# skeskinen/bert.cpp

Hardware: AMD Instinct MI355X
Metric: sentences/sec (seq_len=128) (higher is better)
Workload: dtype f16; 1 GPU; all-MiniLM-L6-v2 f16, batch=256 seq_len=128; per_gpu_batch=256, global_batch=256, seq_len=128, weights=f16, parallelism=dp1 (replicated weights, sharded sentences)

## Files before the change

bert.cpp_amd/csrc/device.h:

```cpp
#pragma once
#include "kernels.h"

#include <cstdio>
#include <type_traits>
#include <utility>

namespace bert_hip {

typedef _Float16 f16x2 __attribute__((ext_vector_type(2)));
typedef _Float16 f16x4 __attribute__((ext_vector_type(4)));
typedef _Float16 f16x8 __attribute__((ext_vector_type(8)));
typedef float f32x2 __attribute__((ext_vector_type(2)));
typedef float f32x4 __attribute__((ext_vector_type(4)));
typedef float f32x8 __attribute__((ext_vector_type(8)));
typedef float f32x16 __attribute__((ext_vector_type(16)));
typedef uint32_t u32x4 __attribute__((ext_vector_type(4)));
typedef uint32_t u32x16 __attribute__((ext_vector_type(16)));
typedef int32_t i32x4 __attribute__((ext_vector_type(4)));
typedef int32_t i32x16 __attribute__((ext_vector_type(16)));

template <int... I, class F>
__device__ __forceinline__ void static_for_impl(std::integer_sequence<int, I...>, F &&f) {
    (f(std::integral_constant<int, I>{}), ...);
}
template <int N, class F>
__device__ __forceinline__ void static_for(F &&f) { static_for_impl(std::make_integer_sequence<int, N>{}, f); }

#define AS_GLOBAL(p) ((const __attribute__((address_space(1))) void *)(p))
#define AS_LDS(p) ((__attribute__((address_space(3))) void *)(p))
template <class T>
using lds_cptr = const __attribute__((address_space(3))) T *;


#ifdef BERT_HIP_TIMELINE
static __device__ unsigned long long g_timeline[1024 * 256];
#define TL_STAMP(i) do { const int tl_i = (i); if (threadIdx.x == 0 && tl_i < 256) g_timeline[(blockIdx.x & 1023) * 256 + tl_i] = __builtin_readcyclecounter(); } while (0)
#define TL_STAMP_AT(sel, i) do { const int tl_i = (i); if ((sel) && tl_i < 256) g_timeline[(blockIdx.x & 1023) * 256 + tl_i] = __builtin_readcyclecounter(); } while (0)
#define TL_REALTIME_AT(sel, i) do { const int tl_i = (i); if ((sel) && tl_i < 256) g_timeline[(blockIdx.x & 1023) * 256 + tl_i] = __builtin_amdgcn_s_memrealtime(); } while (0)
#define TL_DUMP(cond, nstamps) do {                                                                          \
    static int tl_shots = 0;                                                                                  \
    if ((cond) && tl_shots++ == 20) {                                                                         \
        (void)hipDeviceSynchronize();                                                                         \
        static unsigned long long tl_h[1024 * 256];                                                           \
        (void)hipMemcpyFromSymbol(tl_h, HIP_SYMBOL(g_timeline), sizeof(tl_h));                                \
        const int tl_n = (nstamps) < 256 ? (nstamps) : 256;                                                   \
        for (int b : {0, 1, 100, 255}) {                                                                      \
            fprintf(stderr, "timeline wg %3d:", b);                                                           \
            for (int i = 1; i < tl_n; ++i) fprintf(stderr, " %llu", tl_h[b * 256 + i] - tl_h[b * 256 + i - 1]); \
            fprintf(stderr, "  total %llu\n", tl_h[b * 256 + tl_n - 1] - tl_h[b * 256]);                      \
        }                                                                                                     \
    }                                                                                                         \
} while (0)
#define TL_DUMP_RAW(cond, nstamps) do {                                                                      \
    static int tl_shots = 0;                                                                                  \
    if ((cond) && tl_shots++ == 20) {                                                                         \
        (void)hipDeviceSynchronize();                                                                         \
        static unsigned long long tl_h[1024 * 256];                                                           \
        (void)hipMemcpyFromSymbol(tl_h, HIP_SYMBOL(g_timeline), sizeof(tl_h));                                \
        for (int b : {0, 100}) {                                                                              \
            fprintf(stderr, "rawtimeline wg %3d:", b);                                                        \
            for (int i = 0; i < (nstamps); ++i)                                                               \
                fprintf(stderr, " %lld", tl_h[b * 256 + i] ? (long long)(tl_h[b * 256 + i] - tl_h[b * 256]) : -1LL); \
            fprintf(stderr, "\n");                                                                            \
        }                                                                                                     \
    }                                                                                                         \
} while (0)
#else
#define TL_DUMP_RAW(cond, nstamps) do { } while (0)
#define TL_REALTIME_AT(sel, i) do { } while (0)
#define TL_STAMP(i) do { } while (0)
#define TL_STAMP_AT(sel, i) do { } while (0)
#define TL_DUMP(cond, nstamps) do { } while (0)
#endif

__device__ __forceinline__ unsigned lds_addr(const void *p) {
    return (unsigned)(size_t)(__attribute__((address_space(3))) const char *)p;
}
template <bool MEMORY, int OFF, class V = f16x8>
__device__ __forceinline__ V lds_read_b128(unsigned addr) {
    static_assert(sizeof(V) == 16, "ds_read_b128 reads 16 bytes");
    static_assert(OFF >= 0 && OFF < 65536, "ds offset field is 16 bits");
    V v;
    if constexpr (MEMORY) asm volatile("ds_read_b128 %0, %1 offset:%2" : "=v"(v) : "v"(addr), "n"(OFF) : "memory");
    else asm volatile("ds_read_b128 %0, %1 offset:%2" : "=v"(v) : "v"(addr), "n"(OFF));
    return v;
}
template <class V>
__device__ __forceinline__ void landed(V &v) { asm volatile("" : "+v"(v)); }
template <int VM>
__device__ __forceinline__ void dma_barrier() {
    asm volatile("s_waitcnt vmcnt(%0) lgkmcnt(0)\n\ts_barrier" : : "n"(VM) : "memory");
}

__device__ __forceinline__ int off64(int row, int chunk) { return row * 128 + ((chunk ^ ((row >> 1) & 7)) << 4); }

__device__ __forceinline__ float rounded_f32(float v) {
    asm("" : "+v"(v));
    return v;
}

__device__ __forceinline__ void xor32_pair(float &a, float &b) {
    asm("s_nop 1\n\tv_permlane32_swap_b32 %0, %1\n\ts_nop 1" : "+v"(a), "+v"(b));
}
__device__ __forceinline__ f16x8 result_to_operand_fragment(const f16x8 &v) {
    const u32x4 d = __builtin_bit_cast(u32x4, v);
    uint32_t d0 = d[0], d1 = d[1], d2 = d[2], d3 = d[3];
    asm("s_nop 1\n\tv_permlane32_swap_b32 %0, %2\n\tv_permlane32_swap_b32 %1, %3\n\ts_nop 1" : "+v"(d0), "+v"(d1), "+v"(d2), "+v"(d3));
    return __builtin_bit_cast(f16x8, u32x4{d0, d1, d2, d3});
}
constexpr int ctx_edge_offset(int nq) { return nq * 4096 > 80 * 1024 ? nq * 4096 : 80 * 1024; }
__device__ __forceinline__ float xor32_sum(float v) { float a = v, b = v; xor32_pair(a, b); return a + b; }
__device__ __forceinline__ float xor32_max(float v) { float a = v, b = v; xor32_pair(a, b); return __builtin_fmaxf(a, b); }
__device__ __forceinline__ float wave_sum_f32(float v) {
    v = xor32_sum(v);
    v += __builtin_bit_cast(float, __builtin_amdgcn_ds_swizzle(__builtin_bit_cast(int, v), (16 << 10) | 0x1F));
    v += __builtin_bit_cast(float, __builtin_amdgcn_ds_swizzle(__builtin_bit_cast(int, v), (8 << 10) | 0x1F));
    v += __builtin_bit_cast(float, __builtin_amdgcn_ds_swizzle(__builtin_bit_cast(int, v), (4 << 10) | 0x1F));
    v += __builtin_bit_cast(float, __builtin_amdgcn_mov_dpp(__builtin_bit_cast(int, v), 0x4E, 0xF, 0xF, true));
    v += __builtin_bit_cast(float, __builtin_amdgcn_mov_dpp(__builtin_bit_cast(int, v), 0xB1, 0xF, 0xF, true));
    return v;
}

#ifndef BERT_HIP_EXP16
#define BERT_HIP_EXP16 0
#endif
#if BERT_HIP_EXP16
typedef u32x4 sm_arg_t;
typedef u32x4 sm_exp_t;
__device__ __forceinline__ sm_arg_t softmax_args4(float s0, float s1, float s2, float s3, float s4, float s5, float s6, float s7, float sc, float m) {
    uint32_t a0, a1, a2, a3;
    asm("v_fma_mixlo_f16 %0, %4, %12, -%13\n\t"
        "v_fma_mixlo_f16 %1, %6, %12, -%13\n\t"
        "v_fma_mixlo_f16 %2, %8, %12, -%13\n\t"
        "v_fma_mixlo_f16 %3, %10, %12, -%13\n\t"
        "v_fma_mixhi_f16 %0, %5, %12, -%13\n\t"
        "v_fma_mixhi_f16 %1, %7, %12, -%13\n\t"
        "v_fma_mixhi_f16 %2, %9, %12, -%13\n\t"
        "v_fma_mixhi_f16 %3, %11, %12, -%13"
        : "=&v"(a0), "=&v"(a1), "=&v"(a2), "=&v"(a3)
        : "v"(s0), "v"(s1), "v"(s2), "v"(s3), "v"(s4), "v"(s5), "v"(s6), "v"(s7), "s"(sc), "v"(m));
    return u32x4{a0, a1, a2, a3};
}
__device__ __forceinline__ sm_exp_t softmax_exp4(sm_arg_t a) {
    uint32_t p0, p1, p2, p3;
    asm("v_exp_f16_e32 %0, %4\n\t"
        "v_exp_f16_e32 %1, %5\n\t"
        "v_exp_f16_e32 %2, %6\n\t"
        "v_exp_f16_e32 %3, %7\n\t"
        "v_exp_f16_sdwa %0, %4 dst_sel:WORD_1 dst_unused:UNUSED_PRESERVE src0_sel:WORD_1\n\t"
        "v_exp_f16_sdwa %1, %5 dst_sel:WORD_1 dst_unused:UNUSED_PRESERVE src0_sel:WORD_1\n\t"
        "v_exp_f16_sdwa %2, %6 dst_sel:WORD_1 dst_unused:UNUSED_PRESERVE src0_sel:WORD_1\n\t"
        "v_exp_f16_sdwa %3, %7 dst_sel:WORD_1 dst_unused:UNUSED_PRESERVE src0_sel:WORD_1\n\t"
        "s_nop 0"
        : "=&v"(p0), "=&v"(p1), "=&v"(p2), "=&v"(p3)
        : "v"(a[0]), "v"(a[1]), "v"(a[2]), "v"(a[3]));
    return u32x4{p0, p1, p2, p3};
}
__device__ __forceinline__ void softmax_sum4(sm_exp_t p, float &psum) {
    const f16x2 one = {(_Float16)1.0f, (_Float16)1.0f};
#pragma unroll
    for (int e = 0; e < 4; ++e) {
        const uint32_t pe = p[e];
        psum = __builtin_amdgcn_fdot2(__builtin_bit_cast(f16x2, pe), one, psum, false);
    }
}
__device__ __forceinline__ f16x8 softmax_pack(sm_exp_t p) { return __builtin_bit_cast(f16x8, p); }
#else
typedef f32x8 sm_arg_t;
typedef f32x8 sm_exp_t;
__device__ __forceinline__ sm_arg_t softmax_args4(float s0, float s1, float s2, float s3, float s4, float s5, float s6, float s7, float sc, float m) {
    const float s[8] = {s0, s1, s2, s3, s4, s5, s6, s7};
    f32x8 a;
#pragma unroll
    for (int e = 0; e < 8; ++e) a[e] = __builtin_fmaf(s[e], sc, -m);
    return a;
}
__device__ __forceinline__ sm_exp_t softmax_exp4(sm_arg_t a) {
    f32x8 p;
#pragma unroll
    for (int e = 0; e < 8; ++e) p[e] = __builtin_amdgcn_exp2f(a[e]);
    return p;
}
__device__ __forceinline__ void softmax_sum4(sm_exp_t p, float &psum) {
#pragma unroll
    for (int e = 0; e < 8; ++e) psum += p[e];
}
__device__ __forceinline__ f16x8 softmax_pack(sm_exp_t p) {
    f16x8 pf;
#pragma unroll
    for (int e = 0; e < 8; ++e) pf[e] = (_Float16)p[e];
    return pf;
}
#endif
__device__ __forceinline__ f16x8 softmax_p8(float s0, float s1, float s2, float s3, float s4, float s5, float s6, float s7, float sc,
                                            float m, float &psum) {
    const sm_exp_t p = softmax_exp4(softmax_args4(s0, s1, s2, s3, s4, s5, s6, s7, sc, m));
    softmax_sum4(p, psum);
    return softmax_pack(p);
}
__device__ __forceinline__ f16x2 gelu_pk16h(f16x2 xh) {
    const float c1 = -2.0f * 0.79788456080286535588f * 1.44269504088896340736f;
    const f16x2 C1 = {(_Float16)c1, (_Float16)c1}, C2 = {(_Float16)(c1 * 0.044715f), (_Float16)(c1 * 0.044715f)};
    const f16x2 one = {(_Float16)1.0f, (_Float16)1.0f};
    const f16x2 t = (xh * xh * C2 + C1) * xh;
    const f16x2 e = {(_Float16)__builtin_exp2f16(t[0]), (_Float16)__builtin_exp2f16(t[1])};
    const f16x2 d = e + one;
    const f16x2 r = {(_Float16)__builtin_amdgcn_rcph(d[0]), (_Float16)__builtin_amdgcn_rcph(d[1])};
    return xh * r;
}
__device__ __forceinline__ f16x2 gelu_pk16(float a0, float a1) { return gelu_pk16h(f16x2{(_Float16)a0, (_Float16)a1}); }

__device__ __forceinline__ void layernorm_scale(float s1, float s2, float inv_h, float &rstd, float &nmr) {
    const float mean = s1 * inv_h, ex2 = s2 * inv_h;
    const float t = fmaxf(__builtin_fmaf(-mean, mean, ex2), 0.f) + 1e-5f;
    const float r = __builtin_amdgcn_rsqf(t);
    rstd = r * __builtin_fmaf(-0.5f * t, r * r, 1.5f);
    nmr = -mean * rstd;
}

struct RawBlock { uint4 q; unsigned sc; };
template <int WT>
__device__ __forceinline__ RawBlock q4_load_block(const uint4 *qs, const void *sc, size_t index) {
    RawBlock r;
    r.q = qs[index];
    r.sc = WT == GW_Q4_0 ? (unsigned)((const unsigned short *)sc)[index] : ((const unsigned *)sc)[index];
    return r;
}
template <int WT>
struct Q4Expansion {
    f16x2 d2, m2, off;
    unsigned magic, sel01, sel23;
    __device__ __forceinline__ explicit Q4Expansion(unsigned sc) {
        if (WT == GW_Q4_0) {
            const _Float16 d = __builtin_bit_cast(_Float16, (unsigned short)(sc & 0xffffu));
            d2 = (f16x2){d, d};
            m2 = (f16x2){(_Float16)0, (_Float16)0};
        } else {
            const f16x2 dm = __builtin_bit_cast(f16x2, sc);
            d2 = (f16x2){dm[0], dm[0]};
            m2 = (f16x2){dm[1], dm[1]};
        }
        unsigned offb;
        asm volatile("v_mov_b32 %0, 0x64646464" : "=v"(magic));
        asm volatile("s_mov_b32 %0, 0x04010400" : "=s"(sel01));
        asm volatile("s_mov_b32 %0, 0x04030402" : "=s"(sel23));
        if (WT == GW_Q4_0) asm volatile("s_mov_b32 %0, 0x64086408" : "=s"(offb));
        else asm volatile("s_mov_b32 %0, 0x64006400" : "=s"(offb));
        off = __builtin_bit_cast(f16x2, offb);
    }
    template <bool Q_FIRST>
    __device__ __forceinline__ void four(unsigned word, bool high, unsigned &o0, unsigned &o1) const {
        const unsigned n4 = (high ? (word >> 4) : word) & 0x0f0f0f0fu;
        f16x2 v0 = __builtin_bit_cast(f16x2, __builtin_amdgcn_perm(magic, n4, sel01)) - off;
        f16x2 v1 = __builtin_bit_cast(f16x2, __builtin_amdgcn_perm(magic, n4, sel23)) - off;
        if (WT == GW_Q4_0) { v0 = v0 * d2; v1 = v1 * d2; }
        else if (Q_FIRST) { v0 = __builtin_elementwise_fma(v0, d2, m2); v1 = __builtin_elementwise_fma(v1, d2, m2); }
        else { v0 = __builtin_elementwise_fma(d2, v0, m2); v1 = __builtin_elementwise_fma(d2, v1, m2); }
        o0 = __builtin_bit_cast(unsigned, v0);
        o1 = __builtin_bit_cast(unsigned, v1);
    }
};
template <int WT, bool PERM, class ChunkPtr>
__device__ __forceinline__ void q4_expand_block(const RawBlock &r, ChunkPtr chunk_ptr) {
    const unsigned w[4] = {r.q.x, r.q.y, r.q.z, r.q.w};
    const Q4Expansion<WT> x(r.sc);
#pragma unroll
    for (int h = 0; h < 2; ++h)
#pragma unroll
        for (int pr = 0; pr < 2; ++pr) {
            uint4 out;
            x.template four<false>(w[PERM ? pr : 2 * pr], h, out.x, out.y);
            x.template four<false>(w[PERM ? pr + 2 : 2 * pr + 1], h, out.z, out.w);
            *(uint4 *)chunk_ptr(2 * h + pr) = out;
        }
}
template <int WT>
__device__ __forceinline__ uint4 q4_expand_chunk(const RawBlock &r, int c) {
    const Q4Expansion<WT> x(r.sc);
    const bool high = c >= 2;
    const unsigned w0 = (c & 1) ? r.q.z : r.q.x, w1 = (c & 1) ? r.q.w : r.q.y;
    uint4 out;
    x.template four<true>(w0, high, out.x, out.y);
    x.template four<true>(w1, high, out.z, out.w);
    return out;
}

template <bool PAIR, int NT, class Run, class Landed>
__device__ __forceinline__ void layernorm_runs_of(Run x, Landed landed, const float *gamma, const float *beta, int hi, f16x4 (&y)[4 * NT][4]) {
    constexpr int H = 128 * NT;
    constexpr int AHEAD = 2;
    f32x4 gv[AHEAD + 1][4], bv[AHEAD + 1][4];
    auto request = [&](int n) __attribute__((always_inline)) {
#pragma unroll
        for (int g = 0; g < 4; ++g) {
            gv[n % (AHEAD + 1)][g] = *(const f32x4 *)(gamma + 32 * n + 8 * g + 4 * hi);
            bv[n % (AHEAD + 1)][g] = *(const f32x4 *)(beta + 32 * n + 8 * g + 4 * hi);
        }
    };
#pragma unroll
    for (int n = 0; n < AHEAD; ++n) request(n);
    landed();
    float s1 = 0.f, s2 = 0.f;
    auto add_block = [&](float &a1, float &a2, int n) __attribute__((always_inline)) {
#pragma unroll
        for (int g = 0; g < 4; ++g) {
            const f32x4 v = x(n, g);
#pragma unroll
            for (int e = 0; e < 4; ++e) { a1 += v[e]; a2 = __builtin_fmaf(v[e], v[e], a2); }
        }
    };
    if constexpr (PAIR) {
        float t1[2] = {0.f, 0.f}, t2[2] = {0.f, 0.f};
#pragma unroll
        for (int role = 0; role < 2; ++role)
#pragma unroll
            for (int b = 0; b < 2 * NT; ++b) add_block(t1[role], t2[role], (b >> 1) * 4 + role * 2 + (b & 1));
#pragma unroll
        for (int role = 0; role < 2; ++role) { t1[role] += __shfl_xor(t1[role], 32); t2[role] += __shfl_xor(t2[role], 32); }
        s1 = t1[0] + t1[1]; s2 = t2[0] + t2[1];
    } else {
#pragma unroll
        for (int n = 0; n < 4 * NT; ++n) add_block(s1, s2, n);
        s1 += __shfl_xor(s1, 32); s2 += __shfl_xor(s2, 32);
    }
    float rstd, nmr;
    layernorm_scale(s1, s2, 1.0f / H, rstd, nmr);
    asm volatile("" ::: "memory");
#pragma unroll
    for (int n = 0; n < 4 * NT; ++n) {
        if (n + AHEAD < 4 * NT) request(n + AHEAD);
        __builtin_amdgcn_sched_barrier(0);
#pragma unroll
        for (int g = 0; g < 4; ++g) {
            const f32x4 v = x(n, g), gq = gv[n % (AHEAD + 1)][g], bq = bv[n % (AHEAD + 1)][g];
            f32x4 r;
#pragma unroll
            for (int e = 0; e < 4; ++e) r[e] = __builtin_fmaf(v[e], gq[e] * rstd, __builtin_fmaf(gq[e], nmr, bq[e]));
            asm("" : "+v"(r));
#pragma unroll
            for (int e = 0; e < 4; ++e) y[n][g][e] = (_Float16)r[e];
        }
        __builtin_amdgcn_sched_barrier(0);
    }
}

template <bool PAIR, int NT>
__device__ __forceinline__ void layernorm_runs(const float *row, const float *gamma, const float *beta, int hi, f16x4 (&y)[4 * NT][4]) {
    f32x4 x[4 * NT][4];
#pragma unroll
    for (int n = 0; n < 4 * NT; ++n)
#pragma unroll
        for (int g = 0; g < 4; ++g) x[n][g] = *(const f32x4 *)(row + 32 * n + 8 * g + 4 * hi);
    layernorm_runs_of<PAIR, NT>([&](int n, int g) __attribute__((always_inline)) { return x[n][g]; }, [] {}, gamma, beta, hi, y);
}

}
```

bert.cpp_amd/csrc/engine.h:

```cpp
#pragma once
#include <hip/hip_runtime.h>

#include <cstdint>
#include <functional>
#include <memory>
#include <string>
#include <vector>

#include "kernels.h"
#include "model_file.h"
#include "options.h"
#include "profiler.h"
#include "weights.h"

namespace bert_hip {

class Engine {
public:
    static Engine *create(const ModelFile &mf, int device, std::string &err);
    ~Engine();

    int eval_packed_host(const int32_t *tokens, const int32_t *cu_seqlens, int n_sentences, float *embeddings,
                         std::string &err, float *d_embeddings = nullptr);
    int eval_packed_device(const int32_t *d_tokens, const int32_t *d_cu, int n_sentences, int n_tokens, int max_len,
                           float *d_out, hipStream_t stream, float *d_hidden, std::string &err,
                           const int2 *d_windows = nullptr, int n_windows = 0, int window_slots = 0,
                           int pool_mode = -1);
    static void build_windows(const int32_t *cu_seqlens, int n_sentences, std::vector<int2> &windows, int slots);
    int eval_hidden(const int32_t *tokens, int n_tokens, float *hidden, float *embedding, std::string &err);

    bool reserve(int n_tokens, int n_sentences, std::string &err);
    int check(std::string &err);
    void set_option(const std::string &key, const std::string &value);
    void profile_enable(bool on) { prof_.enable(on); }
    std::string profile_report();
    void timed_launch(const char *name, double flops, hipStream_t s, const std::function<void()> &f);

    const HParams &hparams() const { return hp_; }
    const EngineOptions &options() const { return opt_; }
    int device() const { return device_; }
    hipStream_t stream() const { return stream_; }

private:
    Engine() = default;
    bool ensure_workspace(int t_pad, int n_sentences, std::string &err);

    enum class Route { F32, LATENCY, ONE_LAUNCH, FOLDED, LAYERED };
    enum class Family { GEMM256, MFMA, NAIVE, F32 };
    struct LayerPlan {
        bool qkv2 = false;
        bool tail = false;
        bool planes = false;
        Family qkv = Family::NAIVE, o = Family::NAIVE, ffi = Family::NAIVE, ffo = Family::NAIVE;
    };
    struct Plan {
        const int32_t *tokens, *cu;
        int B, T, max_len, t_pad, slots, pool_mode;
        float *out, *hidden;
        hipStream_t s;
        const int2 *windows;
        int n_windows;
        Route route = Route::LAYERED;
        bool build_windows = false;
        const int *n_windows_dev = nullptr;
        std::vector<LayerPlan> layers;
    };
    Plan plan(const int32_t *d_tokens, const int32_t *d_cu, int B, int T, int max_len, float *d_out, hipStream_t s, float *d_hidden,
              const int2 *d_windows, int n_windows, int slots, int pool_mode) const;
    bool forward_f32(const Plan &p, std::string &err);
    void forward_latency(const Plan &p);
    void forward_one_launch(const Plan &p);
    bool forward_folded(const Plan &p, std::string &err);
    bool forward_layers(const Plan &p, std::string &err);
    bool gemm(const Plan &p, const char *name, Family f, const GemmWeightStore &W, const void *A, const float *bias, const void *resid, void *C,
              int epi, std::string &err, const GemmLnFold *ln = nullptr);
    void attention(const Plan &p);
    void tap(const Plan &p, int idx);
    template <class F> void timed(const char *name, double flops, hipStream_t s, F &&f) { prof_.timed(name, flops, s, f); }

    HParams hp_;
    int device_ = 0;
    EngineOptions opt_;
    std::unique_ptr<ModelWeights> w_;
    LaunchProfiler prof_;

    DevBuf x_, qkv_, ctx_, y_, ff_, v32_, d_tokens_, d_cu_, d_out_, d_hidden_, status_, windows_;
    DevBuf ln_stats1_, ln_stats2_, ln_rows1_, ln_rows2_;
    hipStream_t stream_ = nullptr;
    hipEvent_t busy_ = nullptr;
    struct HostSlot {
        char *h_in = nullptr, *d_in_host = nullptr;
        float *h_out = nullptr, *d_out_host = nullptr;
        size_t h_in_cap = 0, h_out_cap = 0;
        DevBuf d_in, d_out;
        hipEvent_t done = nullptr;
    } slot_[2];
};

}
```

bert.cpp_amd/csrc/engine.hip:

```cpp
#include "engine.h"

#include <algorithm>
#include <cstdio>
#include <cstdlib>
#include <chrono>
#include <cstring>
#include <system_error>
#include <thread>

namespace bert_hip {

Engine *Engine::create(const ModelFile &mf, int device, std::string &err) {
    int ndev = 0;
    if (hipGetDeviceCount(&ndev) != hipSuccess || ndev <= 0) {
        err = "no HIP device available (this library needs an AMD GPU; there is no CPU fallback)";
        return nullptr;
    }
    if (device < 0 || device >= ndev) { err = "HIP device ordinal " + std::to_string(device) + " out of range"; return nullptr; }
    std::unique_ptr<Engine> e(new Engine);
    e->hp_ = mf.hp;
    e->device_ = device;
    if (hipSetDevice(e->device_) != hipSuccess) { err = "hipSetDevice failed"; return nullptr; }
    hipDeviceProp_t prop;
    if (hipGetDeviceProperties(&prop, e->device_) != hipSuccess) { err = "hipGetDeviceProperties failed"; return nullptr; }
    if (strncmp(prop.gcnArchName, "gfx950", 6) != 0) {
        err = std::string("unsupported GPU architecture '") + prop.gcnArchName + "' (kernels are built for gfx950 / MI355X only)";
        return nullptr;
    }
    e->opt_ = EngineOptions::from_env(mf.hp);
    LoadOptions lo;
    lo.naive = e->opt_.gemm_naive; lo.expand_q4 = e->opt_.q4_expand; lo.ln_fold = e->opt_.ln_fold;
    e->w_ = ModelWeights::load(mf, lo, err);
    if (!e->w_ || !e->status_.alloc(16, err)) return nullptr;
    if (hipStreamCreateWithFlags(&e->stream_, hipStreamNonBlocking) != hipSuccess) { err = "hipStreamCreate failed"; return nullptr; }
    if (hipEventCreateWithFlags(&e->busy_, hipEventDisableTiming) != hipSuccess) { err = "hipEventCreate failed"; return nullptr; }
    return e.release();
}

Engine::~Engine() {
    (void)hipSetDevice(device_);
    (void)hipDeviceSynchronize();
    for (auto &sl : slot_) {
        if (sl.h_in) (void)hipHostFree(sl.h_in);
        if (sl.h_out) (void)hipHostFree(sl.h_out);
        if (sl.done) (void)hipEventDestroy(sl.done);
    }
    if (busy_) (void)hipEventDestroy(busy_);
    if (stream_) (void)hipStreamDestroy(stream_);
}

bool Engine::reserve(int n_tokens, int n_sentences, std::string &err) {
    HIP_OK(hipSetDevice(device_), err, false);
    if (n_tokens <= 0 || n_sentences <= 0) return true;
    return ensure_workspace((n_tokens + 255) / 256 * 256, n_sentences, err);
}

int Engine::check(std::string &err) {
    HIP_OK(hipSetDevice(device_), err, -1);
    HIP_OK(hipDeviceSynchronize(), err, -1);
    int st = 0;
    HIP_OK(hipMemcpy(&st, status_.p, sizeof(int), hipMemcpyDeviceToHost), err, -1);
    if (st) HIP_OK(hipMemset(status_.p, 0, sizeof(int)), err, -1);
    return st;
}

void Engine::set_option(const std::string &key, const std::string &value) {
    if (key == "profile_replay") { prof_.set_replay(value); return; }
    (void)hipSetDevice(device_);
    if (!test_poison_option(key, ctx_)) opt_.set(key, value, w_->naive_images(), w_->fold_images);
}

bool Engine::ensure_workspace(int t_pad, int n_sentences, std::string &err) {
    const size_t H = hp_.n_embd, I = hp_.n_intermediate, tp = (size_t)t_pad;
    const size_t es = w_->f32_file ? 4 : 2;
    return x_.ensure(tp * H * es, err) && qkv_.ensure(tp * 3 * H * es, err) && ctx_.ensure(tp * H * es, err) &&
           y_.ensure(tp * H * es, err) && ff_.ensure(tp * I * es, err) && v32_.ensure((size_t)std::max(128, std::min(t_pad, (opt_.latency_tokens + 255) / 256 * 256)) * H * 4, err) &&
           d_out_.ensure((size_t)n_sentences * H * 4, err) &&
           windows_.ensure((size_t)n_sentences * sizeof(int2), err) &&
           (!(H > 384 && H % 256 == 0) || (ln_stats1_.ensure(tp * (2 * H / 256) * 8, err) && ln_stats2_.ensure(tp * (2 * H / 256) * 8, err) &&
                                           ln_rows1_.ensure(tp * 16, err) && ln_rows2_.ensure(tp * 16, err)));
}

void Engine::timed_launch(const char *name, double flops, hipStream_t s, const std::function<void()> &f) { timed(name, flops, s, f); }

std::string Engine::profile_report() {
    (void)hipSetDevice(device_);
    (void)hipDeviceSynchronize();
    return prof_.report();
}

void Engine::build_windows(const int32_t *cu, int B, std::vector<int2> &windows, int slot) {
    windows.clear();
    int first = 0, fill = 0;
    for (int b = 0; b < B; ++b) {
        const int n = cu[b + 1] - cu[b];
        if (b > first && fill + n > 128) {
            windows.push_back(make_int2(first, b - first));
            first = b; fill = 0;
        }
        fill = (fill + n + slot - 1) & ~(slot - 1);
    }
    if (B > first) windows.push_back(make_int2(first, B - first));
}

int Engine::eval_packed_device(const int32_t *d_tokens, const int32_t *d_cu, int B, int T, int max_len, float *d_out,
                               hipStream_t s, float *d_hidden, std::string &err, const int2 *d_windows, int n_windows, int slots_in,
                               int pool_mode_in) {
    if (B <= 0 || T <= 0) return 0;
    const int slots = slots_in ? slots_in : window_slots();
    const int pool_mode = pool_mode_in >= 0 ? pool_mode_in : opt_.pool_mode();
    HIP_OK(hipSetDevice(device_), err, -1);
    if (!ensure_workspace((T + 255) / 256 * 256, B, err)) return -1;
    prof_.begin_pass();
    HIP_OK(hipStreamWaitEvent(s, busy_, 0), err, -1);
    const Plan p = plan(d_tokens, d_cu, B, T, max_len, d_out, s, d_hidden, d_windows, n_windows, slots, pool_mode);
    bool ok = true;
    if (p.route == Route::F32) ok = forward_f32(p, err);
    else {
        const int H = hp_.n_embd;
        timed("embed_ln", 0.0, s, [&] { launch_embed_ln(w_->word_emb.p, w_->type_emb.p, w_->pos_emb.p, w_->table_type, w_->ln_e_w.as<float>(), w_->ln_e_b.as<float>(),
                                                        d_tokens, d_cu, B, T, H, hp_.n_vocab, max_len, x_.as<half_t>(), s); });
        tap(p, 0);
        if (p.build_windows)
            timed("build_windows", 0.0, s, [&] { launch_build_windows(d_cu, B, windows_.as<int2>(), status_.as<int>() + 1, slots, s); });
        switch (p.route) {
            case Route::LATENCY: forward_latency(p); break;
            case Route::ONE_LAUNCH: forward_one_launch(p); break;
            case Route::FOLDED: ok = forward_folded(p, err); break;
            default: ok = forward_layers(p, err); break;
        }
        if (ok && p.route != Route::ONE_LAUNCH)
            timed("pool_normalize", 2.0 * T * H, s, [&] { launch_pool_normalize(x_.as<half_t>(), d_cu, B, H, max_len, status_.as<int>(), d_out, p.pool_mode, s); });
    }
    if (!ok) return -1;
    HIP_OK(hipGetLastError(), err, -1);
    HIP_OK(hipEventRecord(busy_, s), err, -1);
    return 0;
}

Engine::Plan Engine::plan(const int32_t *d_tokens, const int32_t *d_cu, int B, int T, int max_len, float *d_out, hipStream_t s,
                          float *d_hidden, const int2 *d_windows, int n_windows, int slots, int pool_mode) const {
    Plan p{d_tokens, d_cu, B, T, max_len, (T + 255) / 256 * 256, slots, pool_mode, d_out, d_hidden, s, d_windows, n_windows};
    if (w_->f32_file && opt_.f32_exact) { p.route = Route::F32; return p; }
    const int H = hp_.n_embd, nh = hp_.n_head, dh = H / nh, Lz = hp_.n_layer;
    auto family = [&](const GemmWeightStore &W) {
        if (W.mfma_ok && opt_.gemm256 && !opt_.gemm_naive && gemm256_supported(W.w, p.t_pad)) return Family::GEMM256;
        return W.mfma_ok && (!opt_.gemm_naive || !W.w.naive16) ? Family::MFMA : Family::NAIVE;
    };
    p.layers.resize(Lz);
    bool qkv2_shape0 = false, one_launch = true, fold = opt_.ln_fold && H > 384 && H % 256 == 0 && ln_rows2_.p;
    for (int il = 0; il < Lz; ++il) {
        const LayerWeights &L = w_->layers[il];
        LayerPlan &lp = p.layers[il];
        const bool qkv2_shape = qkv_attention2_supported(L.qkv.w, nh, dh, max_len), tail_shape = layer_tail_supported(L.o.w, L.ffi.w, L.ffo.w);
        if (il == 0) qkv2_shape0 = qkv2_shape;
        lp.qkv2 = opt_.qkv2 && !opt_.gemm_naive && !opt_.attn_naive && L.qkv.mfma_ok && qkv2_shape;
        lp.tail = opt_.tail && !opt_.gemm_naive && L.o.mfma_ok && L.ffi.mfma_ok && L.ffo.mfma_ok && tail_shape;
        lp.planes = L.qkv_q4.w.qs && family(L.qkv_q4) == Family::GEMM256;
        lp.qkv = family(lp.planes ? L.qkv_q4 : L.qkv), lp.o = family(L.o), lp.ffi = family(L.ffi), lp.ffo = family(L.ffo);
        one_launch = one_launch && L.qkv.mfma_ok && L.o.mfma_ok && L.ffi.mfma_ok && L.ffo.mfma_ok && L.ffi.w.w16p && L.ffo.w.w16p &&
                     model_kernel_supported(L.qkv.w, L.o.w, L.ffi.w, L.ffo.w, Lz, nh, dh, max_len);
        fold = fold && L.fold_ok && (il ? family(L.qkv_fold) : lp.qkv) == Family::GEMM256 && lp.o == Family::GEMM256 &&
               family(L.ffi_fold) == Family::GEMM256 && lp.ffo == Family::GEMM256 && !(opt_.qkv2 && qkv2_shape) && !(opt_.tail && tail_shape);
    }
    if (d_hidden) one_launch = fold = false;
    const bool fused_windows = p.layers[0].qkv2, latency_call = opt_.latency && T <= opt_.latency_tokens;
    one_launch = one_launch && fused_windows && opt_.one_launch && opt_.tail && !latency_call;
    const bool full_windows = (long long)B * 128 == T;
    const int spw = qkv_attention2_sentences_per_window(max_len, slots);
    if (!d_windows && fused_windows &&
        (4ll * ((B + spw - 1) / spw) * 128 > 5 * ((long long)T + (long long)(slots / 2) * B) || (one_launch && opt_.one_launch == 2 && spw > 1 && !full_windows))) {
        p.build_windows = true;
        p.windows = windows_.as<int2>();
        p.n_windows_dev = status_.as<int>() + 1;
        p.n_windows = qkv_attention2_max_windows(B, T, slots);
    }
    bool one_launch_pays = full_windows || opt_.one_launch == 2;
    if (!one_launch_pays && !p.build_windows) one_launch_pays = (d_windows || spw == 1) && 100ll * T >= 95ll * 128 * (d_windows ? n_windows : B);
    const LayerWeights &L0 = w_->layers[0];
    const bool skinny = latency_call && opt_.tail && opt_.qkv2 && !opt_.gemm_naive && !opt_.attn_naive && max_len <= 128 && (dh == 32 || dh == 64) &&
                        skinny_layer_supported(L0.qkv.w, L0.o.w, L0.ffi.w, L0.ffo.w) && qkv2_shape0;
    p.route = skinny ? Route::LATENCY : one_launch && one_launch_pays ? Route::ONE_LAUNCH : fold ? Route::FOLDED : Route::LAYERED;
    return p;
}

bool Engine::gemm(const Plan &p, const char *name, Family f, const GemmWeightStore &W, const void *A, const float *bias, const void *resid,
                  void *C, int epi, std::string &err, const GemmLnFold *ln) {
    static const char *const kernel[] = {"gemm256", "gemm_mfma", "gemm_naive", "gemm_f32"};
    prof_.count_family(std::string("family:") + kernel[(int)f] + (f == Family::GEMM256 || f == Family::MFMA ? (W.w.type == GW_F16 ? "_f16" : "_q4") : ""));
    const half_t *a = (const half_t *)A, *r = (const half_t *)resid;
    bool ok = !(ln && ln->flags) || f == Family::GEMM256;
    if (ok)
        timed(name, 2.0 * p.T * W.w.N * W.w.K, p.s, [&] {
            if (f == Family::F32) launch_f32_gemm((const float *)A, W.w.w32, bias, (const float *)resid, (float *)C, p.T, W.w.N, W.w.K, epi, p.s);
            else if (f == Family::GEMM256) ok = launch_gemm256(W.w, a, bias, r, (half_t *)C, p.t_pad, epi, p.s, ln);
            else if (f == Family::MFMA) launch_gemm_mfma(W.w, a, bias, r, (half_t *)C, p.t_pad, epi, p.s);
            else launch_gemm_naive(W.w, a, bias, r, (half_t *)C, p.T, epi, p.s);
        });
    if (!ok) err = std::string(name) + ": no " + kernel[(int)f] + " kernel for LayerNorm-folding flags " + std::to_string(ln->flags) + ", epilogue " + std::to_string(epi);
    return ok;
}

void Engine::attention(const Plan &p) {
    const int H = hp_.n_embd, nh = hp_.n_head, dh = H / nh;
    half_t *qkv = qkv_.as<half_t>(), *ctx = ctx_.as<half_t>();
    timed("attention", 4.0 * p.T * p.max_len * H, p.s, [&] {
        if (opt_.attn_naive || !launch_attention_mfma(qkv, p.cu, p.B, nh, dh, p.max_len, ctx, p.s)) launch_attention_naive(qkv, p.cu, p.B, nh, dh, p.max_len, ctx, p.s);
    });
}

void Engine::tap(const Plan &p, int idx) {
    const size_t n = (size_t)p.T * hp_.n_embd;
    if (p.hidden && p.route == Route::F32) (void)hipMemcpyAsync(p.hidden + idx * n, x_.p, n * 4, hipMemcpyDeviceToDevice, p.s);
    else if (p.hidden) launch_f16_to_f32(x_.as<half_t>(), p.hidden + idx * n, n, p.s);
}

void Engine::forward_latency(const Plan &p) {
    const int H = hp_.n_embd, I = hp_.n_intermediate, tb = (p.T + 31) / 32, Lz = hp_.n_layer;
    half_t *x = x_.as<half_t>(), *qkv = qkv_.as<half_t>(), *ctx = ctx_.as<half_t>(), *y = y_.as<half_t>(), *ff = ff_.as<half_t>();
    float *v32 = v32_.as<float>();
    for (int il = 0; il < Lz; ++il) {
        const LayerWeights &L = w_->layers[il];
        const LayerWeights *P = il ? &w_->layers[il - 1] : nullptr;
        timed("skinny_qkv", 2.0 * p.T * 3 * H * H, p.s, [&] {
            launch_skinny_gemm(0, L.qkv.w, x, P ? v32 : nullptr, P ? P->ln_out_w.as<float>() : nullptr, P ? P->ln_out_b.as<float>() : nullptr,
                               x, L.qkv_b.as<float>(), nullptr, qkv, nullptr, tb, p.s);
        });
        attention(p);
        timed("skinny_proj", 2.0 * p.T * H * H, p.s, [&] {
            launch_skinny_gemm(1, L.o.w, ctx, nullptr, nullptr, nullptr, nullptr, L.o_b.as<float>(), x, nullptr, v32, tb, p.s);
        });
        timed("skinny_ffn_up", 2.0 * p.T * H * I, p.s, [&] {
            launch_skinny_gemm(2, L.ffi.w, nullptr, v32, L.ln_att_w.as<float>(), L.ln_att_b.as<float>(), y, L.ffi_b.as<float>(), nullptr, ff, nullptr, tb, p.s);
        });
        timed("skinny_ffn_down", 2.0 * p.T * H * I, p.s, [&] {
            launch_skinny_gemm(3, L.ffo.w, ff, nullptr, nullptr, nullptr, nullptr, L.ffo_b.as<float>(), y, nullptr, v32, tb, p.s);
        });
        if (il + 1 == Lz || p.hidden)
            timed("skinny_layernorm", 0.0, p.s, [&] { launch_skinny_layernorm(v32, L.ln_out_w.as<float>(), L.ln_out_b.as<float>(), x, tb, H, p.s); });
        tap(p, il + 1);
    }
}

void Engine::forward_one_launch(const Plan &p) {
    const int H = hp_.n_embd, I = hp_.n_intermediate;
    ModelLayerWeights mw[MODEL_MAX_LAYERS];
    for (int il = 0; il < hp_.n_layer; ++il) {
        const LayerWeights &L = w_->layers[il];
        mw[il] = {&L.qkv.w, &L.o.w, &L.ffi.w, &L.ffo.w, L.qkv_b.as<float>(), L.o_b.as<float>(), L.ln_att_w.as<float>(), L.ln_att_b.as<float>(),
                  L.ffi_b.as<float>(), L.ffo_b.as<float>(), L.ln_out_w.as<float>(), L.ln_out_b.as<float>()};
    }
    timed("model_kernel", hp_.n_layer * (2.0 * p.T * 3 * H * H + 4.0 * p.T * p.max_len * H + 2.0 * p.T * H * H + 4.0 * p.T * H * I), p.s, [&] {
        launch_model_kernel(mw, hp_.n_layer, x_.as<half_t>(), ctx_.as<half_t>(), p.cu, p.B, p.T, p.windows, p.n_windows, p.n_windows_dev, hp_.n_head,
                            p.out, p.max_len, status_.as<int>(), p.pool_mode, p.slots, p.s);
    });
}

bool Engine::forward_folded(const Plan &p, std::string &err) {
    const int H = hp_.n_embd, P = 2 * H / 256;
    const Family G = Family::GEMM256;
    half_t *x = x_.as<half_t>(), *qkv = qkv_.as<half_t>(), *ctx = ctx_.as<half_t>(), *y = y_.as<half_t>(), *ff = ff_.as<half_t>();
    float2 *st1 = ln_stats1_.as<float2>(), *st2 = ln_stats2_.as<float2>();
    float4 *rows1 = ln_rows1_.as<float4>(), *rows2 = ln_rows2_.as<float4>();
    for (int il = 0; il < hp_.n_layer; ++il) {
        const LayerWeights &L = w_->layers[il];
        GemmLnFold ln;
        if (il == 0) {
            if (!gemm(p, "gemm_qkv", G, p.layers[0].planes ? L.qkv_q4 : L.qkv, x, L.qkv_b.as<float>(), nullptr, qkv, EPI_BIAS, err)) return false;
        } else {
            ln.flags = GemmLnFold::IN; ln.rows_in = rows2; ln.waug = L.qkv_waug.as<half_t>();
            if (!gemm(p, "gemm_qkv", G, L.qkv_fold, x, nullptr, nullptr, qkv, EPI_BIAS, err, &ln)) return false;
        }
        attention(p);
        ln = GemmLnFold(); ln.flags = GemmLnFold::STATS | (il ? GemmLnFold::RES : 0); ln.stats = st1; ln.rows_res = rows2; ln.gb = L.o_gb.as<unsigned>();
        if (!gemm(p, "gemm_attn_out", G, L.o, ctx, L.o_b.as<float>(), x, y, EPI_BIAS_RESID, err, &ln)) return false;
        timed("ln_rows_finalize", 0.0, p.s, [&] { launch_ln_rows_finalize(st1, P, p.t_pad, H, rows1, p.s); });
        ln = GemmLnFold(); ln.flags = GemmLnFold::IN; ln.rows_in = rows1; ln.waug = L.ffi_waug.as<half_t>();
        if (!gemm(p, "gemm_ffn_up", G, L.ffi_fold, y, nullptr, nullptr, ff, EPI_BIAS_GELU, err, &ln)) return false;
        ln = GemmLnFold(); ln.flags = GemmLnFold::STATS | GemmLnFold::RES; ln.stats = st2; ln.rows_res = rows1; ln.gb = L.ffo_gb.as<unsigned>();
        if (!gemm(p, "gemm_ffn_down", G, L.ffo, ff, L.ffo_b.as<float>(), y, x, EPI_BIAS_RESID, err, &ln)) return false;
        timed("ln_rows_finalize", 0.0, p.s, [&] { launch_ln_rows_finalize(st2, P, p.t_pad, H, rows2, p.s); });
        if (il + 1 == hp_.n_layer)
            timed("layernorm", 0.0, p.s, [&] { launch_layernorm(x, L.ln_out_w.as<float>(), L.ln_out_b.as<float>(), p.T, H, p.s); });
    }
    return true;
}

bool Engine::forward_layers(const Plan &p, std::string &err) {
    const int H = hp_.n_embd, I = hp_.n_intermediate;
    half_t *x = x_.as<half_t>(), *qkv = qkv_.as<half_t>(), *ctx = ctx_.as<half_t>(), *y = y_.as<half_t>(), *ff = ff_.as<half_t>();
    for (int il = 0; il < hp_.n_layer; ++il) {
        const LayerWeights &L = w_->layers[il];
        const LayerPlan &lp = p.layers[il];
        if (lp.qkv2) {
            timed("qkv_attention2", 2.0 * p.T * L.qkv.w.N * L.qkv.w.K + 4.0 * p.T * p.max_len * H, p.s, [&] {
                launch_qkv_attention2(L.qkv.w, x, L.qkv_b.as<float>(), p.cu, p.B, p.windows, p.n_windows, p.n_windows_dev, p.max_len, hp_.n_head, p.slots, ctx, p.s);
            });
        } else {
            if (!gemm(p, "gemm_qkv", lp.qkv, lp.planes ? L.qkv_q4 : L.qkv, x, L.qkv_b.as<float>(), nullptr, qkv, EPI_BIAS, err)) return false;
            attention(p);
        }
        if (lp.tail) {
            timed("layer_tail", 2.0 * p.T * H * H + 4.0 * p.T * H * I, p.s, [&] {
                launch_layer_tail(L.o.w, L.ffi.w, L.ffo.w, ctx, x, L.o_b.as<float>(), L.ln_att_w.as<float>(), L.ln_att_b.as<float>(), L.ffi_b.as<float>(),
                                  L.ffo_b.as<float>(), L.ln_out_w.as<float>(), L.ln_out_b.as<float>(), x, p.t_pad, p.s);
            });
        } else {
            if (!gemm(p, "gemm_attn_out", lp.o, L.o, ctx, L.o_b.as<float>(), x, y, EPI_BIAS_RESID, err)) return false;
            timed("layernorm", 0.0, p.s, [&] { launch_layernorm(y, L.ln_att_w.as<float>(), L.ln_att_b.as<float>(), p.T, H, p.s); });
            if (!gemm(p, "gemm_ffn_up", lp.ffi, L.ffi, y, L.ffi_b.as<float>(), nullptr, ff, EPI_BIAS_GELU, err) ||
                !gemm(p, "gemm_ffn_down", lp.ffo, L.ffo, ff, L.ffo_b.as<float>(), y, x, EPI_BIAS_RESID, err)) return false;
            timed("layernorm", 0.0, p.s, [&] { launch_layernorm(x, L.ln_out_w.as<float>(), L.ln_out_b.as<float>(), p.T, H, p.s); });
        }
        tap(p, il + 1);
    }
    return true;
}

bool Engine::forward_f32(const Plan &p, std::string &err) {
    const int H = hp_.n_embd, nh = hp_.n_head, dh = H / nh;
    const Family F = Family::F32;
    float *x = x_.as<float>(), *qkv = qkv_.as<float>(), *ctx = ctx_.as<float>(), *y = y_.as<float>(), *ff = ff_.as<float>();
    timed("embed_ln", 0.0, p.s, [&] {
        launch_f32_embed_ln(w_->word_emb.as<float>(), w_->type_emb.as<float>(), w_->pos_emb.as<float>(), w_->ln_e_w.as<float>(), w_->ln_e_b.as<float>(), p.tokens,
                            p.cu, p.B, p.T, H, hp_.n_vocab, x, p.s);
    });
    tap(p, 0);
    for (int il = 0; il < hp_.n_layer; ++il) {
        const LayerWeights &L = w_->layers[il];
        if (!gemm(p, "gemm_qkv", F, L.qkv, x, L.qkv_b.as<float>(), nullptr, qkv, EPI_BIAS, err)) return false;
        timed("attention", 4.0 * p.T * p.max_len * H, p.s, [&] { launch_f32_attention(qkv, p.cu, p.B, nh, dh, p.max_len, ctx, p.s); });
        if (!gemm(p, "gemm_attn_out", F, L.o, ctx, L.o_b.as<float>(), x, y, EPI_BIAS_RESID, err)) return false;
        timed("layernorm", 0.0, p.s, [&] { launch_f32_layernorm(y, L.ln_att_w.as<float>(), L.ln_att_b.as<float>(), p.T, H, p.s); });
        if (!gemm(p, "gemm_ffn_up", F, L.ffi, y, L.ffi_b.as<float>(), nullptr, ff, EPI_BIAS_GELU, err) ||
            !gemm(p, "gemm_ffn_down", F, L.ffo, ff, L.ffo_b.as<float>(), y, x, EPI_BIAS_RESID, err)) return false;
        timed("layernorm", 0.0, p.s, [&] { launch_f32_layernorm(x, L.ln_out_w.as<float>(), L.ln_out_b.as<float>(), p.T, H, p.s); });
        tap(p, il + 1);
    }
    timed("pool_normalize", 2.0 * p.T * H, p.s, [&] { launch_f32_pool_normalize(x, p.cu, p.B, H, p.max_len, status_.as<int>(), p.out, p.pool_mode, p.s); });
    return true;
}

static bool ensure_pinned(void **p, size_t *cap, size_t need, std::string &err) {
    if (need <= *cap) return true;
    if (*p) (void)hipHostFree(*p);
    *p = nullptr; *cap = 0;
    need += need / 4;
    HIP_OK(hipHostMalloc(p, need, hipHostMallocDefault), err, false);
    *cap = need;
    return true;
}

static void copy_rows_out(float *dst, const float *src, size_t bytes) {
    constexpr size_t PART_MIN = (size_t)1 << 20;
    constexpr int MAX_PARTS = 4;
    const int parts = (int)std::min<size_t>(MAX_PARTS, bytes / PART_MIN);
    if (parts <= 1) { memcpy(dst, src, bytes); return; }
    const size_t each = (bytes / parts + 4095) & ~(size_t)4095;
    std::thread helpers[MAX_PARTS - 1];
    size_t inline_from = each;
    for (int k = 1; k < parts; ++k) {
        const size_t off = (size_t)k * each, n = std::min(each, bytes - std::min(bytes, off));
        if (n == 0) break;
        try {
            helpers[k - 1] = std::thread([=] { memcpy((char *)dst + off, (const char *)src + off, n); });
            inline_from = off + n;
        } catch (const std::system_error &) {
            break;
        }
    }
    memcpy(dst, src, std::min(each, bytes));
    if (inline_from < bytes) memcpy((char *)dst + inline_from, (const char *)src + inline_from, bytes - inline_from);
    for (auto &h : helpers)
        if (h.joinable()) h.join();
}

int Engine::eval_packed_host(const int32_t *tokens, const int32_t *cu, int B, float *embeddings, std::string &err,
                             float *d_embeddings) {
    if (B <= 0) return 0;
#ifdef BERT_HIP_HOST_TRACE
    auto now = [] { return std::chrono::duration<double, std::milli>(std::chrono::steady_clock::now().time_since_epoch()).count(); };
    const double t_call = now();
    double t_mark = t_call;
    auto lap = [&](const char *what, size_t i) { const double t = now(); fprintf(stderr, "[host] chunk %zu %-10s %.3f ms\n", i, what, t - t_mark); t_mark = t; };
#define HOST_LAP(what, i) lap(what, i)
#else
#define HOST_LAP(what, i) do { } while (0)
#endif
    HIP_OK(hipSetDevice(device_), err, -1);
    const int H = hp_.n_embd;
    struct Chunk { int b0, b1, max_len; };
    std::vector<Chunk> chunks;
    size_t max_T = 0, max_nb = 0;
    for (int b0 = 0; b0 < B;) {
        int b1 = b0 + 1, max_len = cu[b0 + 1] - cu[b0];
        while (b1 < B && cu[b1 + 1] - cu[b0] <= opt_.chunk_tokens) { max_len = std::max(max_len, cu[b1 + 1] - cu[b1]); ++b1; }
        chunks.push_back({b0, b1, max_len});
        max_T = std::max(max_T, (size_t)(cu[b1] - cu[b0]));
        max_nb = std::max(max_nb, (size_t)(b1 - b0));
        b0 = b1;
    }
    const int n_slots = chunks.size() > 1 ? 2 : 1;
    auto pad16 = [](size_t n) { return (n + 15) & ~(size_t)15; };
    const size_t in_bytes = pad16(max_T * 4) + pad16((max_nb + 1) * 4) + pad16(max_nb * sizeof(int2));
    for (int i = 0; i < n_slots; ++i) {
        HostSlot &sl = slot_[i];
        const size_t in_cap = sl.h_in_cap;
        if (!ensure_pinned((void **)&sl.h_in, &sl.h_in_cap, in_bytes + 16, err)) return -1;
        if (sl.h_in_cap != in_cap || !sl.d_in_host) HIP_OK(hipHostGetDevicePointer((void **)&sl.d_in_host, sl.h_in, 0), err, -1);
        const size_t out_cap = sl.h_out_cap;
        if (!ensure_pinned((void **)&sl.h_out, &sl.h_out_cap, max_nb * H * 4, err)) return -1;
        if (sl.h_out_cap != out_cap || !sl.d_out_host)
            HIP_OK(hipHostGetDevicePointer((void **)&sl.d_out_host, sl.h_out, 0), err, -1);
        if (!sl.d_in.ensure(in_bytes + 16, err) || (d_embeddings && !sl.d_out.ensure(max_nb * H * 4, err))) return -1;
        if (!sl.done) HIP_OK(hipEventCreateWithFlags(&sl.done, hipEventDisableTiming), err, -1);
    }
    if (!ensure_workspace((int)((max_T + 255) / 256 * 256), (int)max_nb, err)) return -1;
    HOST_LAP("prepared", (size_t)0);

    auto unpack = [&](size_t i) -> bool {
        HostSlot &sl = slot_[i & 1];
        if (hipEventSynchronize(sl.done) != hipSuccess) { err = "hipEventSynchronize failed"; return false; }
        HOST_LAP("wait", i);
        if (!d_embeddings) {
            const size_t bytes = (size_t)(chunks[i].b1 - chunks[i].b0) * H * 4;
            if (i + 1 == chunks.size()) copy_rows_out(embeddings + (size_t)chunks[i].b0 * H, sl.h_out, bytes);
            else memcpy(embeddings + (size_t)chunks[i].b0 * H, sl.h_out, bytes);
        }
        HOST_LAP("copy-out", i);
        return true;
    };
    auto fail = [&]() { (void)hipStreamSynchronize(stream_); return -1; };
    std::vector<int2> windows;
    const int slots = window_slots();
    const int pool_mode = opt_.pool_mode();
    for (size_t i = 0; i < chunks.size(); ++i) {
        HostSlot &sl = slot_[i & 1];
        const int b0 = chunks[i].b0, nb = chunks[i].b1 - b0, T = cu[chunks[i].b1] - cu[b0];
        const size_t off_cu = pad16((size_t)T * 4), off_w = off_cu + pad16((size_t)(nb + 1) * 4);
        int32_t *h_cu = (int32_t *)(sl.h_in + off_cu);
        memcpy(sl.h_in, tokens + cu[b0], (size_t)T * 4);
        for (int j = 0; j <= nb; ++j) h_cu[j] = cu[b0 + j] - cu[b0];
        int n_windows = 0;
        if (chunks[i].max_len <= 128) {
            build_windows(h_cu, nb, windows, slots);
            n_windows = (int)windows.size();
            memcpy(sl.h_in + off_w, windows.data(), windows.size() * sizeof(int2));
        }
        const size_t staged = off_w + (size_t)n_windows * sizeof(int2);
        HOST_LAP("staged", i);
        if (opt_.stage_kernel && staged <= ((size_t)256 << 10)) {
            launch_stage_copy(sl.d_in_host, sl.d_in.p, staged, stream_);
        } else if (hipMemcpyAsync(sl.d_in.p, sl.h_in, staged, hipMemcpyHostToDevice, stream_) != hipSuccess) {
            err = "hipMemcpyAsync (ids) failed";
            return fail();
        }
        const char *d_in = (const char *)sl.d_in.p;
        float *out = d_embeddings ? sl.d_out.as<float>() : sl.d_out_host;
        if (eval_packed_device((const int32_t *)d_in, (const int32_t *)(d_in + off_cu), nb, T, chunks[i].max_len, out, stream_, nullptr, err,
                               n_windows ? (const int2 *)(d_in + off_w) : nullptr, n_windows, slots, pool_mode) != 0)
            return fail();
        if ((d_embeddings && hipMemcpyAsync(d_embeddings + (size_t)b0 * H, sl.d_out.p, (size_t)nb * H * 4, hipMemcpyDeviceToDevice, stream_) != hipSuccess) ||
            hipEventRecord(sl.done, stream_) != hipSuccess) {
            err = "hipMemcpyAsync (embeddings) failed";
            return fail();
        }
        HOST_LAP("queued", i);
        if (i >= 1 && !unpack(i - 1)) return fail();
    }
    if (!unpack(chunks.size() - 1)) return fail();
#undef HOST_LAP
    return 0;
}

int Engine::eval_hidden(const int32_t *tokens, int N, float *hidden, float *embedding, std::string &err) {
    HIP_OK(hipSetDevice(device_), err, -1);
    const int H = hp_.n_embd, L = hp_.n_layer;
    int32_t cu[2] = {0, N};
    if (!d_tokens_.ensure((size_t)N * 4, err) || !d_cu_.ensure(8, err)) return -1;
    if (!d_hidden_.ensure((size_t)(L + 1) * N * H * 4, err)) return -1;
    const int t_pad = (N + 255) / 256 * 256;
    if (!ensure_workspace(t_pad, 1, err)) return -1;
    HIP_OK(hipMemcpy(d_tokens_.p, tokens, (size_t)N * 4, hipMemcpyHostToDevice), err, -1);
    HIP_OK(hipMemcpy(d_cu_.p, cu, 8, hipMemcpyHostToDevice), err, -1);
    if (eval_packed_device(d_tokens_.as<int32_t>(), d_cu_.as<int32_t>(), 1, N, N, d_out_.as<float>(), stream_,
                           d_hidden_.as<float>(), err) != 0)
        return -1;
    HIP_OK(hipStreamSynchronize(stream_), err, -1);
    if (hidden) HIP_OK(hipMemcpy(hidden, d_hidden_.p, (size_t)(L + 1) * N * H * 4, hipMemcpyDeviceToHost), err, -1);
    if (embedding) HIP_OK(hipMemcpy(embedding, d_out_.p, (size_t)H * 4, hipMemcpyDeviceToHost), err, -1);
    return 0;
}

}
```

bert.cpp_amd/csrc/kernels.h:

```cpp
#pragma once
#include <hip/hip_runtime.h>
#include <hip/hip_ext.h>

#include <atomic>
#include <cstdint>
#include <thread>

namespace bert_hip {

typedef _Float16 half_t;

constexpr int GEMM_BM = 128;
constexpr int GEMM_BN = 128;
constexpr int GEMM_BK = 64;

enum Epilogue : int { EPI_BIAS = 0, EPI_BIAS_GELU = 1, EPI_BIAS_RESID = 2 };
enum GemmWType : int { GW_F16 = 0, GW_Q4_0 = 1, GW_Q4_1 = 2 };

struct GemmWeight {
    int N = 0, K = 0, N_pad = 0;
    int type = GW_F16;
    const half_t *w16 = nullptr;
    const uint4 *qs = nullptr;
    const void *sc = nullptr;
    const half_t *naive16 = nullptr;
    const half_t *w16p = nullptr;
    const float *w32 = nullptr;
};

void launch_gemm_mfma(const GemmWeight &W, const half_t *A, const float *bias, const half_t *resid, half_t *C,
                      int M_pad, int epilogue, hipStream_t stream);
bool gemm256_supported(const GemmWeight &W, int M_pad);
struct GemmLnFold {
    enum : int { IN = 1, RES = 2, STATS = 4 };
    int flags = 0;
    const float4 *rows_in = nullptr;
    const half_t *waug = nullptr;
    const float4 *rows_res = nullptr;
    const unsigned *gb = nullptr;
    float2 *stats = nullptr;
};
bool launch_gemm256(const GemmWeight &W, const half_t *A, const float *bias, const half_t *resid, half_t *C, int M_pad,
                    int epilogue, hipStream_t stream, const GemmLnFold *ln = nullptr);
void launch_ln_rows_finalize(const float2 *stats, int P, int T, int H, float4 *rows, hipStream_t stream);
bool layer_tail_supported(const GemmWeight &Wo, const GemmWeight &W1, const GemmWeight &W2);
void launch_layer_tail(const GemmWeight &Wo, const GemmWeight &W1, const GemmWeight &W2, const half_t *ctx, const half_t *x,
                       const float *bo, const float *g1, const float *be1, const float *b1, const float *b2,
                       const float *g2, const float *be2, half_t *out, int M_pad, hipStream_t stream);
constexpr int MODEL_MAX_LAYERS = 12;
struct ModelLayerWeights {
    const GemmWeight *Wqkv, *Wo, *W1, *W2;
    const float *bqkv, *bo, *g1, *be1, *b1, *b2, *g2, *be2;
};
bool model_kernel_supported(const GemmWeight &Wqkv, const GemmWeight &Wo, const GemmWeight &W1, const GemmWeight &W2, int n_layer,
                            int n_head, int d_head, int max_len);
void launch_model_kernel(const ModelLayerWeights *layers, int n_layer, half_t *x, half_t *ctx, const int32_t *cu_seqlens, int n_sentences,
                         int n_tokens, const int2 *groups, int n_groups, const int *n_groups_dev, int n_head, float *pooled, int max_len,
                         int *status, int pool_mode, int slots, hipStream_t stream);
bool skinny_layer_supported(const GemmWeight &Wqkv, const GemmWeight &Wo, const GemmWeight &W1, const GemmWeight &W2);
void launch_skinny_gemm(int mode, const GemmWeight &W, const half_t *A, const float *V, const float *gamma, const float *beta,
                        half_t *ln_out, const float *bias, const half_t *resid, half_t *out16, float *out32, int n_token_blocks,
                        hipStream_t stream);
void launch_skinny_layernorm(const float *v, const float *gamma, const float *beta, half_t *out, int n_token_blocks, int H,
                             hipStream_t stream);
void launch_gemm_naive(const GemmWeight &W, const half_t *A, const float *bias, const half_t *resid, half_t *C,
                       int M, int epilogue, hipStream_t stream);

void launch_embed_ln(const void *word, const void *type, const void *pos, int table_type, const float *gamma,
                     const float *beta, const int32_t *tokens, const int32_t *cu_seqlens, int n_sentences, int T,
                     int H, int n_vocab, int max_len, half_t *out, hipStream_t stream);

void launch_layernorm(half_t *x, const float *gamma, const float *beta, int T, int H, hipStream_t stream);

bool launch_attention_mfma(const half_t *qkv, const int32_t *cu_seqlens, int n_sentences, int n_head, int d_head,
                           int max_len, half_t *out, hipStream_t stream);
void launch_attention_naive(const half_t *qkv, const int32_t *cu_seqlens, int n_sentences, int n_head, int d_head,
                            int max_len, half_t *out, hipStream_t stream);

bool qkv_attention2_supported(const GemmWeight &Wqkv, int n_head, int d_head, int max_len);
int qkv_attention2_sentences_per_window(int max_len, int slots);
void launch_qkv_attention2(const GemmWeight &Wqkv, const half_t *x, const float *bias, const int32_t *cu_seqlens,
                           int n_sentences, const int2 *groups, int n_groups, const int *n_groups_dev, int max_len, int n_head,
                           int slots, half_t *out, hipStream_t stream);
void launch_build_windows(const int32_t *cu_seqlens, int n_sentences, int2 *windows, int *n_windows, int slots, hipStream_t stream);
int qkv_attention2_max_windows(int n_sentences, int n_tokens, int slots);
int window_slots();
void set_window_slots(int slots);

constexpr int POOL_CLS = 1, POOL_RAW = 2;
void launch_pool_normalize(const half_t *x, const int32_t *cu_seqlens, int n_sentences, int H, int max_len, int *status,
                           float *out, int pool_mode, hipStream_t stream);

constexpr int MAX_HIP_DEVICES = 64;
typedef std::atomic<int> DeviceFlags[MAX_HIP_DEVICES];
inline int current_device_slot() {
    int d = 0;
    (void)hipGetDevice(&d);
    return d & (MAX_HIP_DEVICES - 1);
}
inline bool first_launch_on_device(DeviceFlags &seen) {
    std::atomic<int> &f = seen[current_device_slot()];
    int expected = 0;
    if (f.load(std::memory_order_acquire) == 2) return false;
    if (f.compare_exchange_strong(expected, 1, std::memory_order_acq_rel)) return true;
    while (f.load(std::memory_order_acquire) != 2) std::this_thread::yield();
    return false;
}
inline void mark_configured(DeviceFlags &seen) { seen[current_device_slot()].store(2, std::memory_order_release); }
template <class F>
inline void configure_once(DeviceFlags &seen, F &&opt_in) {
    if (first_launch_on_device(seen)) { opt_in(); mark_configured(seen); }
}

struct LaunchTiming { hipEvent_t start, stop; int launches; };
inline thread_local LaunchTiming *tl_launch_timing = nullptr;
#define BERT_LAUNCH(kernel, grid, block, lds, stream, ...)                                                                     \
    do {                                                                                                                      \
        if (::bert_hip::tl_launch_timing) {                                                                                   \
            ++::bert_hip::tl_launch_timing->launches;                                                                         \
            hipExtLaunchKernelGGL(kernel, grid, block, lds, stream, ::bert_hip::tl_launch_timing->start,                      \
                                  ::bert_hip::tl_launch_timing->stop, 0, __VA_ARGS__);                                        \
        } else hipLaunchKernelGGL(kernel, grid, block, lds, stream, __VA_ARGS__);                                             \
    } while (0)

void launch_f32_embed_ln(const float *word, const float *type, const float *pos, const float *gamma, const float *beta, const int32_t *tokens,
                         const int32_t *cu_seqlens, int n_sentences, int T, int H, int n_vocab, float *out, hipStream_t stream);
void launch_f32_gemm(const float *A, const float *W, const float *bias, const float *resid, float *C, int M, int N, int K, int epilogue,
                     hipStream_t stream);
void launch_f32_attention(const float *qkv, const int32_t *cu_seqlens, int n_sentences, int n_head, int d_head, int max_len, float *out,
                          hipStream_t stream);
void launch_f32_layernorm(float *x, const float *gamma, const float *beta, int T, int H, hipStream_t stream);
void launch_f32_pool_normalize(const float *x, const int32_t *cu_seqlens, int n_sentences, int H, int max_len, int *status, float *out,
                               int pool_mode, hipStream_t stream);

void launch_stage_copy(const void *mapped_src, void *dst, size_t bytes, hipStream_t stream);

void launch_f16_to_f32(const half_t *src, float *dst, size_t n, hipStream_t stream);

}
```

bert.cpp_amd/csrc/misc_kernels.hip:

```cpp
#include "device.h"
#include "pool_normalize.h"

#include <algorithm>

namespace bert_hip {

__device__ __forceinline__ float table_elem(const void *tab, int type, int H, int r, int e) {
    if (type == 0) return ((const float *)tab)[(size_t)r * H + e];
    if (type == 1) return (float)((const half_t *)tab)[(size_t)r * H + e];
    const int bs = type == 2 ? 18 : 20;
    const unsigned char *blk = (const unsigned char *)tab + ((size_t)r * (H / 32) + e / 32) * bs;
    const int i = e & 31;
    const float d = (float)*(const half_t *)blk;
    const unsigned char byte = blk[(type == 2 ? 2 : 4) + (i & 15)];
    const int q = i < 16 ? (byte & 0x0F) : (byte >> 4);
    if (type == 2) return (float)(q - 8) * d;
    const float m = (float)*(const half_t *)(blk + 2);
    return (float)q * d + m;
}

__device__ __forceinline__ void table_pair(const void *tab, int type, int H, int r, int e, float &a, float &b) {
    if (type == 0) {
        const float2 v = *(const float2 *)((const float *)tab + (size_t)r * H + e);
        a = v.x; b = v.y;
    } else if (type == 1) {
        const f16x2 v = *(const f16x2 *)((const half_t *)tab + (size_t)r * H + e);
        a = (float)v[0]; b = (float)v[1];
    } else {
        a = table_elem(tab, type, H, r, e);
        b = table_elem(tab, type, H, r, e + 1);
    }
}

template <int NJ>
__global__ __launch_bounds__(256) void embed_ln_kernel(const void *word, const void *type, const void *pos,
                                                       int table_type, const float *gamma, const float *beta,
                                                       const int32_t *__restrict__ tokens,
                                                       const int32_t *__restrict__ cu_seqlens, int n_sentences,
                                                       int T, int H, int n_vocab, half_t *__restrict__ out) {
    const int t = blockIdx.x * 4 + __builtin_amdgcn_readfirstlane(threadIdx.x >> 6), lane = threadIdx.x & 63;
    if (t >= T) return;
    int lo = 0, hi = n_sentences;
    while (hi - lo > 1) {
        const int mid = (lo + hi) >> 1;
        if (cu_seqlens[mid] <= t) lo = mid; else hi = mid;
    }
    const int p = t - cu_seqlens[lo];
    int id = tokens[t];
    id = id < 0 ? 0 : (id >= n_vocab ? n_vocab - 1 : id);

    float v[NJ][2];
    float sum = 0.f;
#pragma unroll
    for (int j = 0; j < NJ; ++j) {
        const int e = 2 * lane + 128 * j;
        v[j][0] = v[j][1] = 0.f;
        if (e < H) {
            float w0, w1, t0, t1, p0, p1;
            table_pair(word, table_type, H, id, e, w0, w1);
            table_pair(type, table_type, H, 0, e, t0, t1);
            table_pair(pos, table_type, H, p, e, p0, p1);
            v[j][0] = p0 + (t0 + w0);
            v[j][1] = p1 + (t1 + w1);
            sum += v[j][0] + v[j][1];
        }
    }
    const float mean = wave_sum_f32(sum) / H;
    float sq = 0.f;
#pragma unroll
    for (int j = 0; j < NJ; ++j) {
        const int e = 2 * lane + 128 * j;
        if (e < H) {
            v[j][0] -= mean; v[j][1] -= mean;
            sq += v[j][0] * v[j][0] + v[j][1] * v[j][1];
        }
    }
    const float rstd = 1.0f / sqrtf(wave_sum_f32(sq) / H + 1e-5f);
#pragma unroll
    for (int j = 0; j < NJ; ++j) {
        const int e = 2 * lane + 128 * j;
        if (e < H) {
            f16x2 o;
            o[0] = (_Float16)(gamma[e] * (v[j][0] * rstd) + beta[e]);
            o[1] = (_Float16)(gamma[e + 1] * (v[j][1] * rstd) + beta[e + 1]);
            *(f16x2 *)(out + (size_t)t * H + e) = o;
        }
    }
}

template <int TT>
__device__ __forceinline__ void table_run8(const void *tab, int H, int r, int e0, float (&v)[8]) {
    if (TT == 0) {
        const float4 a = *(const float4 *)((const float *)tab + (size_t)r * H + e0);
        const float4 b = *(const float4 *)((const float *)tab + (size_t)r * H + e0 + 4);
        v[0] = a.x; v[1] = a.y; v[2] = a.z; v[3] = a.w; v[4] = b.x; v[5] = b.y; v[6] = b.z; v[7] = b.w;
    } else if (TT == 1) {
        const f16x8 h = *(const f16x8 *)((const half_t *)tab + (size_t)r * H + e0);
#pragma unroll
        for (int i = 0; i < 8; ++i) v[i] = (float)h[i];
    } else {
        constexpr int bs = TT == 2 ? 18 : 20, qo = TT == 2 ? 2 : 4;
        const unsigned char *blk = (const unsigned char *)tab + ((size_t)r * (H / 32) + (e0 >> 5)) * bs;
        const int off = e0 & 31;
        const float d = (float)*(const half_t *)blk;
        const float m = TT == 3 ? (float)*(const half_t *)(blk + 2) : 0.f;
        unsigned short q16[4];
#pragma unroll
        for (int i = 0; i < 4; ++i) q16[i] = *(const unsigned short *)(blk + qo + (off & 15) + 2 * i);
#pragma unroll
        for (int i = 0; i < 8; ++i) {
            const int byte = (q16[i >> 1] >> (8 * (i & 1))) & 0xff, q = off < 16 ? (byte & 0x0F) : (byte >> 4);
            v[i] = TT == 2 ? (float)(q - 8) * d : (float)q * d + m;
        }
    }
}
template <int TT, int NC, bool SEARCH>
__global__ __launch_bounds__(256) void embed_ln_rows_kernel(const void *word, const void *type, const void *pos,
                                                            const float *__restrict__ gamma, const float *__restrict__ beta,
                                                            const int32_t *__restrict__ tokens,
                                                            const int32_t *__restrict__ cu_seqlens, int n_sentences, int T,
                                                            int H, int n_vocab, half_t *__restrict__ out) {
    const int lane = threadIdx.x & 63;
    int p = blockIdx.x * 4 + __builtin_amdgcn_readfirstlane(threadIdx.x >> 6);
    int t;
    if constexpr (SEARCH) {
        t = p;
        if (t >= T) return;
        int lo = 0, hi = n_sentences;
        while (hi - lo > 1) {
            const int mid = (lo + hi) >> 1;
            if (cu_seqlens[mid] <= t) lo = mid; else hi = mid;
        }
        p = t - cu_seqlens[lo];
    } else {
        const int b = blockIdx.y;
        const int tok0 = cu_seqlens[b], n = cu_seqlens[b + 1] - tok0;
        if (p >= n) return;
        t = tok0 + p;
    }
    int id = tokens[t];
    id = id < 0 ? 0 : (id >= n_vocab ? n_vocab - 1 : id);
    float v[NC][8];
    float sum = 0.f;
#pragma unroll
    for (int j = 0; j < NC; ++j) {
        const int e0 = 8 * (lane + 64 * j);
#pragma unroll
        for (int i = 0; i < 8; ++i) v[j][i] = 0.f;
        if (e0 < H) {
            float w[8], ty[8], ps[8];
            table_run8<TT>(word, H, id, e0, w);
            table_run8<TT>(type, H, 0, e0, ty);
            table_run8<TT>(pos, H, p, e0, ps);
#pragma unroll
            for (int i = 0; i < 8; ++i) { v[j][i] = ps[i] + (ty[i] + w[i]); sum += v[j][i]; }
        }
    }
    const float mean = wave_sum_f32(sum) / H;
    float sq = 0.f;
#pragma unroll
    for (int j = 0; j < NC; ++j)
        if (8 * (lane + 64 * j) < H)
#pragma unroll
            for (int i = 0; i < 8; ++i) { v[j][i] -= mean; sq += v[j][i] * v[j][i]; }
    const float rstd = 1.0f / sqrtf(wave_sum_f32(sq) / H + 1e-5f);
#pragma unroll
    for (int j = 0; j < NC; ++j) {
        const int e0 = 8 * (lane + 64 * j);
        if (e0 < H) {
            const float4 g0 = *(const float4 *)(gamma + e0), g1 = *(const float4 *)(gamma + e0 + 4);
            const float4 b0 = *(const float4 *)(beta + e0), b1 = *(const float4 *)(beta + e0 + 4);
            const float gg[8] = {g0.x, g0.y, g0.z, g0.w, g1.x, g1.y, g1.z, g1.w};
            const float bb[8] = {b0.x, b0.y, b0.z, b0.w, b1.x, b1.y, b1.z, b1.w};
            f16x8 o;
#pragma unroll
            for (int i = 0; i < 8; ++i) o[i] = (_Float16)(gg[i] * (v[j][i] * rstd) + bb[i]);
            *(f16x8 *)(out + (size_t)t * H + e0) = o;
        }
    }
}

void launch_embed_ln(const void *word, const void *type, const void *pos, int table_type, const float *gamma,
                     const float *beta, const int32_t *tokens, const int32_t *cu_seqlens, int n_sentences, int T,
                     int H, int n_vocab, int max_len, half_t *out, hipStream_t stream) {
    if (T <= 0) return;
    if ((table_type <= 1 ? H % 8 == 0 : H % 32 == 0) && table_type <= 3 && H <= 1024 && max_len > 0) {
        const bool search = n_sentences > 65535 || 2ll * ((max_len + 3) / 4) * n_sentences > 3ll * ((T + 3) / 4);
        const dim3 g2 = search ? dim3((T + 3) / 4) : dim3((max_len + 3) / 4, n_sentences), b2(256);
#define EMBR(TT, NC) do { \
            if (search) BERT_LAUNCH((embed_ln_rows_kernel<TT, NC, true>), g2, b2, 0, stream, word, type, pos, gamma, beta, tokens, \
                                           cu_seqlens, n_sentences, T, H, n_vocab, out); \
            else BERT_LAUNCH((embed_ln_rows_kernel<TT, NC, false>), g2, b2, 0, stream, word, type, pos, gamma, beta, tokens, \
                                    cu_seqlens, n_sentences, T, H, n_vocab, out); } while (0)
        if (table_type == 0) { if (H <= 512) EMBR(0, 1); else EMBR(0, 2); }
        else if (table_type == 1) { if (H <= 512) EMBR(1, 1); else EMBR(1, 2); }
        else if (table_type == 2) { if (H <= 512) EMBR(2, 1); else EMBR(2, 2); }
        else { if (H <= 512) EMBR(3, 1); else EMBR(3, 2); }
#undef EMBR
        return;
    }
    const dim3 grid((T + 3) / 4), block(256);
    const int nj = (H + 127) / 128;
#define EMB(NJ) BERT_LAUNCH(embed_ln_kernel<NJ>, grid, block, 0, stream, word, type, pos, table_type, gamma, \
                                   beta, tokens, cu_seqlens, n_sentences, T, H, n_vocab, out)
    if (nj <= 1) EMB(1); else if (nj <= 3) EMB(3); else if (nj <= 6) EMB(6); else if (nj <= 8) EMB(8); else EMB(32);
#undef EMB
}

template <int NJ>
__global__ __launch_bounds__(256) void layernorm_kernel(half_t *x, const float *gamma, const float *beta, int T, int H) {
    const int t = blockIdx.x * 4 + (threadIdx.x >> 6), lane = threadIdx.x & 63;
    if (t >= T) return;
    half_t *row = x + (size_t)t * H;
    float v[NJ][2];
    float sum = 0.f;
#pragma unroll
    for (int j = 0; j < NJ; ++j) {
        const int e = 2 * lane + 128 * j;
        if (e < H) {
            const f16x2 h2 = *(const f16x2 *)(row + e);
            v[j][0] = (float)h2[0]; v[j][1] = (float)h2[1];
        } else { v[j][0] = 0.f; v[j][1] = 0.f; }
        sum += v[j][0] + v[j][1];
    }
    const float mean = wave_sum_f32(sum) / H;
    float sq = 0.f;
#pragma unroll
    for (int j = 0; j < NJ; ++j) {
        const int e = 2 * lane + 128 * j;
        if (e < H) {
            v[j][0] -= mean; v[j][1] -= mean;
            sq += v[j][0] * v[j][0] + v[j][1] * v[j][1];
        }
    }
    const float rstd = 1.0f / sqrtf(wave_sum_f32(sq) / H + 1e-5f);
#pragma unroll
    for (int j = 0; j < NJ; ++j) {
        const int e = 2 * lane + 128 * j;
        if (e < H) {
            f16x2 o;
            o[0] = (_Float16)(gamma[e] * (v[j][0] * rstd) + beta[e]);
            o[1] = (_Float16)(gamma[e + 1] * (v[j][1] * rstd) + beta[e + 1]);
            *(f16x2 *)(row + e) = o;
        }
    }
}

template <int NC>
__global__ __launch_bounds__(256) void layernorm_rows_kernel(half_t *x, const float *__restrict__ gamma,
                                                             const float *__restrict__ beta, int T, int H) {
    const int t = blockIdx.x * 4 + (threadIdx.x >> 6), lane = threadIdx.x & 63;
    if (t >= T) return;
    half_t *row = x + (size_t)t * H;
    f16x8 h[NC];
#pragma unroll
    for (int j = 0; j < NC; ++j) {
        const int e0 = 8 * (lane + 64 * j);
#pragma unroll
        for (int i = 0; i < 8; ++i) h[j][i] = (_Float16)0.f;
        if (e0 < H) h[j] = *(const f16x8 *)(row + e0);
    }
    float v[NC][8];
    float sum = 0.f;
#pragma unroll
    for (int j = 0; j < NC; ++j)
#pragma unroll
        for (int i = 0; i < 8; ++i) { v[j][i] = (float)h[j][i]; sum += v[j][i]; }
    const float mean = wave_sum_f32(sum) / H;
    float sq = 0.f;
#pragma unroll
    for (int j = 0; j < NC; ++j)
        if (8 * (lane + 64 * j) < H)
#pragma unroll
            for (int i = 0; i < 8; ++i) { v[j][i] -= mean; sq += v[j][i] * v[j][i]; }
    const float rstd = 1.0f / sqrtf(wave_sum_f32(sq) / H + 1e-5f);
#pragma unroll
    for (int j = 0; j < NC; ++j) {
        const int e0 = 8 * (lane + 64 * j);
        if (e0 < H) {
            const float4 g0 = *(const float4 *)(gamma + e0), g1 = *(const float4 *)(gamma + e0 + 4);
            const float4 b0 = *(const float4 *)(beta + e0), b1 = *(const float4 *)(beta + e0 + 4);
            const float gg[8] = {g0.x, g0.y, g0.z, g0.w, g1.x, g1.y, g1.z, g1.w};
            const float bb[8] = {b0.x, b0.y, b0.z, b0.w, b1.x, b1.y, b1.z, b1.w};
            f16x8 o;
#pragma unroll
            for (int i = 0; i < 8; ++i) o[i] = (_Float16)(gg[i] * (v[j][i] * rstd) + bb[i]);
            *(f16x8 *)(row + e0) = o;
        }
    }
}

void launch_layernorm(half_t *x, const float *gamma, const float *beta, int T, int H, hipStream_t stream) {
    if (T <= 0) return;
    if (H % 8 == 0 && H <= 2048) {
        const dim3 grid((T + 3) / 4), block(256);
        if (H <= 512) BERT_LAUNCH(layernorm_rows_kernel<1>, grid, block, 0, stream, x, gamma, beta, T, H);
        else if (H <= 1024) BERT_LAUNCH(layernorm_rows_kernel<2>, grid, block, 0, stream, x, gamma, beta, T, H);
        else BERT_LAUNCH(layernorm_rows_kernel<4>, grid, block, 0, stream, x, gamma, beta, T, H);
        return;
    }
    const dim3 grid((T + 3) / 4), block(256);
    const int nj = (H + 127) / 128;
    if (nj <= 1) BERT_LAUNCH(layernorm_kernel<1>, grid, block, 0, stream, x, gamma, beta, T, H);
    else if (nj <= 3) BERT_LAUNCH(layernorm_kernel<3>, grid, block, 0, stream, x, gamma, beta, T, H);
    else if (nj <= 6) BERT_LAUNCH(layernorm_kernel<6>, grid, block, 0, stream, x, gamma, beta, T, H);
    else if (nj <= 8) BERT_LAUNCH(layernorm_kernel<8>, grid, block, 0, stream, x, gamma, beta, T, H);
    else BERT_LAUNCH(layernorm_kernel<32>, grid, block, 0, stream, x, gamma, beta, T, H);
}

__global__ __launch_bounds__(256) void ln_rows_finalize_kernel(const float2 *__restrict__ stats, int P, int T, float inv_h, float4 *__restrict__ rows) {
    const int t = blockIdx.x * 256 + threadIdx.x;
    if (t >= T) return;
    float s1 = 0.f, s2 = 0.f;
    for (int p = 0; p < P; ++p) { const float2 v = stats[(size_t)t * P + p]; s1 += v.x; s2 += v.y; }
    const float mean = s1 * inv_h, var = fmaxf(s2 * inv_h - mean * mean, 0.f) + 1e-5f;
    const float sd = sqrtf(var), rstd = 1.0f / sd;
    rows[t] = make_float4(rstd, -mean * rstd, -mean, sd);
}

void launch_ln_rows_finalize(const float2 *stats, int P, int T, int H, float4 *rows, hipStream_t stream) {
    if (T <= 0) return;
    BERT_LAUNCH(ln_rows_finalize_kernel, dim3((T + 255) / 256), dim3(256), 0, stream, stats, P, T, 1.0f / H, rows);
}

__global__ __launch_bounds__(256) void pool_normalize_kernel(const half_t *x, const int32_t *cu_seqlens, int H,
                                                             int max_len, int *status, float *out, int pool_mode) {
    extern __shared__ float part[];
    const int b = blockIdx.x;
    const int tok0 = cu_seqlens[b], n = cu_seqlens[b + 1] - tok0;
    pool_normalize_sentence(x, tok0, n, b, H, max_len, status, out, part, (int)threadIdx.x, true, pool_mode);
}

void launch_pool_normalize(const half_t *x, const int32_t *cu_seqlens, int n_sentences, int H, int max_len, int *status,
                           float *out, int pool_mode, hipStream_t stream) {
    if (n_sentences <= 0) return;
    BERT_LAUNCH(pool_normalize_kernel, dim3(n_sentences), dim3(256), (4 * H + 4) * sizeof(float), stream, x,
                       cu_seqlens, H, max_len, status, out, pool_mode);
}

__global__ __launch_bounds__(256) void stage_copy_kernel(const uint4 *__restrict__ src, uint4 *__restrict__ dst, int n16) {
    for (int i = blockIdx.x * 256 + threadIdx.x; i < n16; i += gridDim.x * 256) dst[i] = src[i];
}

void launch_stage_copy(const void *mapped_src, void *dst, size_t bytes, hipStream_t stream) {
    const int n16 = (int)((bytes + 15) / 16);
    if (n16 <= 0) return;
    BERT_LAUNCH(stage_copy_kernel, dim3(std::min(64, (n16 + 255) / 256)), dim3(256), 0, stream, (const uint4 *)mapped_src, (uint4 *)dst, n16);
}

__global__ void f16_to_f32_kernel(const half_t *src, float *dst, size_t n) {
    const size_t i = (size_t)blockIdx.x * 256 + threadIdx.x;
    if (i < n) dst[i] = (float)src[i];
}

void launch_f16_to_f32(const half_t *src, float *dst, size_t n, hipStream_t stream) {
    if (!n) return;
    BERT_LAUNCH(f16_to_f32_kernel, dim3((unsigned)((n + 255) / 256)), dim3(256), 0, stream, src, dst, n);
}

}
```

bert.cpp_amd/csrc/model_kernel.hip:

```cpp
#define BERT_HIP_PHASES_ONLY
#include "qkv_attention2.hip"
#include "layer_tail.hip"
#undef BERT_HIP_PHASES_ONLY
#include "pool_normalize.h"

#include <cstdlib>

namespace bert_hip {

#ifdef BERT_HIP_MODEL_TIMELINE
static __device__ unsigned long long g_tl_model[1024 * 32];
#define MK_STAMP(i) do { const int mk_i = (i); if (threadIdx.x == 0 && mk_i < 32) g_tl_model[(blockIdx.x & 1023) * 32 + mk_i] = __builtin_amdgcn_s_memrealtime(); } while (0)
#else
#define MK_STAMP(i) do { } while (0)
#endif

namespace {

struct ModelLayerArgs {
    const half_t *wqkv, *wo, *w1p, *w2p;
    const float *bqkv, *bo, *g1, *be1, *b1, *b2, *g2, *be2;
};
struct ModelArgs {
    half_t *x, *ctx;
    const int32_t *cu;
    const int2 *groups;
    const int *n_groups;
    int n_layer, n_head, n_sent, I, slot_mask;
    float *pooled;
    int *status;
    int max_len, pool_mode;
    ModelLayerArgs layer[MODEL_MAX_LAYERS];
};

}

template <int NT, bool RAGGED, bool POOL_MODES>
__global__ __launch_bounds__(512, 2) void model_kernel(ModelArgs m) {
    extern __shared__ __attribute__((aligned(16))) char smem[];
    const int window = (int)blockIdx.x;
    int tok0 = window * 128, rows = 128, first = window, count = 1;
    if constexpr (RAGGED) {
        if (m.groups) {
            if (m.n_groups && window >= *m.n_groups) return;
            const int2 g = m.groups[window];
            first = g.x; count = g.y;
        }
        if (count <= 0 || first >= m.n_sent) return;
        tok0 = m.cu[first];
        rows = min(m.cu[first + count] - tok0, 128);
    }
    const int wave_index = __builtin_amdgcn_readfirstlane((int)threadIdx.x >> 6);
    auto thread_id = [&]() __attribute__((always_inline)) {
        int ln = (int)__builtin_amdgcn_mbcnt_hi(~0u, __builtin_amdgcn_mbcnt_lo(~0u, 0u)), w = wave_index;
        asm volatile("" : "+v"(ln), "+s"(w));
        return w * 64 + ln;
    };
    MK_STAMP(0);
    const int n_layer = rows > 0 ? m.n_layer : 0;
    auto window_phase = [&](const ModelLayerArgs &L, auto xregs_tag, const f16x8 *xf, f16x8 *cf) __attribute__((always_inline)) {
        const int tid = thread_id();
        Qkv2Args q;
        q.x = m.x; q.w = L.wqkv; q.qs = nullptr; q.sc = nullptr; q.bias = L.bqkv; q.cu = m.cu; q.groups = RAGGED ? m.groups : nullptr; q.n_groups = nullptr;
        q.out = m.ctx; q.n_head = m.n_head; q.n_sent = m.n_sent; q.spw = 1; q.slot_mask = m.slot_mask;
        qkv_attention2_body<2 * NT, NT, GW_F16, !RAGGED, decltype(xregs_tag)::value, !RAGGED>(q, smem, window, tid, xf, cf);
    };
    auto tail_phase = [&](const ModelLayerArgs &L, f16x8 (&xf)[8 * NT], const f16x8 *cf) __attribute__((always_inline)) {
        const int tid = thread_id();
        TailArgs t;
        t.ctx = m.ctx; t.x = m.x; t.wo = L.wo; t.w1p = L.w1p; t.w2p = L.w2p;
        t.wo_qs = t.w1_qs = t.w2_qs = nullptr; t.wo_sc = t.w1_sc = t.w2_sc = nullptr;
        t.bo = L.bo; t.g1 = L.g1; t.be1 = L.be1; t.b1 = L.b1; t.b2 = L.b2; t.g2 = L.g2; t.be2 = L.be2; t.out = m.x; t.I = m.I;
        layer_tail_body<NT, GW_F16, RAGGED, !RAGGED, !RAGGED>(t, smem, tok0, rows, tid, xf, cf);
    };
    auto hand_over = [&]() __attribute__((always_inline)) {
        __builtin_amdgcn_fence(__ATOMIC_RELEASE, "workgroup");
        asm volatile("s_waitcnt vmcnt(0) lgkmcnt(0)\n\ts_barrier" ::: "memory");
        __builtin_amdgcn_fence(__ATOMIC_ACQUIRE, "workgroup");
    };
    if constexpr (RAGGED) {
        for (int l = 0; l < n_layer; ++l) {
            f16x8 none[8 * NT];
            window_phase(m.layer[l], std::false_type{}, nullptr, nullptr);
            hand_over();
            MK_STAMP(1 + 2 * l);
            tail_phase(m.layer[l], none, nullptr);
            hand_over();
            MK_STAMP(2 + 2 * l);
        }
    } else {
        f16x8 cf[8 * NT];
        if (n_layer > 0) window_phase(m.layer[0], std::false_type{}, nullptr, cf);
        for (int l = 0; l < n_layer; ++l) {
            hand_over();
            MK_STAMP(1 + 2 * l);
            f16x8 xf[8 * NT];
            tail_phase(m.layer[l], xf, cf);
            hand_over();
            MK_STAMP(2 + 2 * l);
            if (l + 1 < n_layer) window_phase(m.layer[l + 1], std::true_type{}, xf, cf);
            else {
#pragma unroll
                for (int q = 0; q < 8 * NT; ++q) asm volatile("" : "=v"(cf[q]));
            }
        }
    }
    if (m.pooled) {
        const int tid = thread_id();
        for (int j = 0; j < count; ++j) {
            const int b = first + j, t0 = m.cu[b];
            int n = m.cu[b + 1] - t0;
            if (!RAGGED && (t0 != tok0 || n != 128)) n = -1;
            if constexpr (POOL_MODES) pool_normalize_sentence(m.x, t0, n, b, 128 * NT, m.max_len, m.status, m.pooled, (float *)smem, tid, tid < 256, m.pool_mode);
            else pool_normalize_sentence<false, false>(m.x, t0, n, b, 128 * NT, m.max_len, m.status, m.pooled, (float *)smem, tid, tid < 256);
            __syncthreads();
        }
    }
    MK_STAMP(1 + 2 * n_layer);
}

bool model_kernel_supported(const GemmWeight &Wqkv, const GemmWeight &Wo, const GemmWeight &W1, const GemmWeight &W2, int n_layer,
                            int n_head, int d_head, int max_len) {
    const int H = n_head * d_head;
    return n_layer <= MODEL_MAX_LAYERS && (H == 256 || H == 384) && max_len >= 1 && max_len <= 128 &&
           Wqkv.type == GW_F16 && Wo.type == GW_F16 && qkv_attention2_supported(Wqkv, n_head, d_head, max_len) && layer_tail_supported(Wo, W1, W2);
}

void launch_model_kernel(const ModelLayerWeights *layers, int n_layer, half_t *x, half_t *ctx, const int32_t *cu_seqlens, int n_sentences,
                         int n_tokens, const int2 *groups, int n_groups, const int *n_groups_dev, int n_head, float *pooled, int max_len,
                         int *status, int pool_mode, int slots, hipStream_t stream) {
    ModelArgs m;
    m.pooled = pooled; m.status = status; m.max_len = max_len; m.pool_mode = pool_mode;
    m.x = x; m.ctx = ctx; m.cu = cu_seqlens; m.groups = groups; m.n_groups = n_groups_dev;
    m.n_layer = n_layer; m.n_head = n_head; m.n_sent = n_sentences; m.I = layers[0].W1->N; m.slot_mask = slots - 1;
    for (int l = 0; l < n_layer; ++l) {
        const ModelLayerWeights &s = layers[l];
        ModelLayerArgs &d = m.layer[l];
        d.wqkv = s.Wqkv->w16; d.wo = s.Wo->w16; d.w1p = s.W1->w16p; d.w2p = s.W2->w16p;
        d.bqkv = s.bqkv; d.bo = s.bo; d.g1 = s.g1; d.be1 = s.be1; d.b1 = s.b1; d.b2 = s.b2; d.g2 = s.g2; d.be2 = s.be2;
    }
    const int H = layers[0].W1->K, KT = H / 64, GB = KT / 2;
    const size_t lds_q = (size_t)3 * GB * Q2_TILE + 2 * (2 * Q2_WIN * 64 + 32 * Q2_VT_LD * 2) + (size_t)2 * H * sizeof(float);
    const size_t lds = std::max(lds_q, layer_tail_lds(H, m.I));
    const bool full = (long long)n_sentences * 128 == n_tokens;
    if (n_head * 32 != H) { fprintf(stderr, "launch_model_kernel: n_head %d x 32 != H %d\n", n_head, H); abort(); }
    const int grid = full || !groups ? n_sentences : n_groups;
    static DeviceFlags configured[8];
    auto go = [&](auto kernel, int which) {
        configure_once(configured[which], [&] { (void)hipFuncSetAttribute((const void *)kernel, hipFuncAttributeMaxDynamicSharedMemorySize, 160 * 1024); });
        BERT_LAUNCH(kernel, dim3(grid), dim3(512), lds, stream, m);
#ifdef BERT_HIP_MODEL_TIMELINE
        static int shots = 0;
        if (grid >= 256 && shots++ == 30) {
            (void)hipDeviceSynchronize();
            static unsigned long long h[1024 * 32];
            (void)hipMemcpyFromSymbol(h, HIP_SYMBOL(g_tl_model), sizeof(h));
            const int nw = grid < 1024 ? grid : 1024, ns = 2 + 2 * n_layer;
            unsigned long long t0 = ~0ull;
            for (int w = 0; w < nw; ++w) t0 = h[w * 32] < t0 ? h[w * 32] : t0;
            fprintf(stderr, "model_kernel timeline, %d workgroups (us after the first workgroup's start: min mean max):\n", nw);
            for (int i = 0; i < ns; ++i) {
                double lo = 1e30, hi = 0, sum = 0;
                for (int w = 0; w < nw; ++w) { const double v = (double)(h[w * 32 + i] - t0) * 0.01; lo = v < lo ? v : lo; hi = v > hi ? v : hi; sum += v; }
                fprintf(stderr, "  stamp %2d: %8.2f %8.2f %8.2f\n", i, lo, sum / nw, hi);
            }
            fprintf(stderr, "  mean phase durations (window, tail) per layer:");
            for (int l = 0; l < n_layer; ++l) {
                double a = 0, b = 0;
                for (int w = 0; w < nw; ++w) { a += (double)(h[w * 32 + 1 + 2 * l] - h[w * 32 + 2 * l]) * 0.01; b += (double)(h[w * 32 + 2 + 2 * l] - h[w * 32 + 1 + 2 * l]) * 0.01; }
                fprintf(stderr, " (%.1f, %.1f)", a / nw, b / nw);
            }
            fprintf(stderr, "\n  mean end per XCD:");
            for (int x = 0; x < 8; ++x) {
                double e = 0; int c = 0;
                for (int w = x; w < nw; w += 8) { e += (double)(h[w * 32 + ns - 1] - t0) * 0.01; ++c; }
                fprintf(stderr, " %.1f", e / c);
            }
            fprintf(stderr, "\n  mean end per eighth of the grid:");
            for (int x = 0; x < 8; ++x) {
                double e = 0; int c = 0;
                for (int w = x * nw / 8; w < (x + 1) * nw / 8; ++w) { e += (double)(h[w * 32 + ns - 1] - t0) * 0.01; ++c; }
                fprintf(stderr, " %.1f", e / c);
            }
            double pl = 0;
            for (int w = 0; w < nw; ++w) pl += (double)(h[w * 32 + 1 + 2 * n_layer] - h[w * 32 + 2 * n_layer]) * 0.01;
            fprintf(stderr, "; pooling %.2f\n", pl / nw);
        }
#endif
    };
    if (pool_mode == 0) {
        if (full) { if (H == 256) go(model_kernel<2, false, false>, 0); else go(model_kernel<3, false, false>, 1); }
        else { if (H == 256) go(model_kernel<2, true, false>, 2); else go(model_kernel<3, true, false>, 3); }
    } else {
        if (full) { if (H == 256) go(model_kernel<2, false, true>, 4); else go(model_kernel<3, false, true>, 5); }
        else { if (H == 256) go(model_kernel<2, true, true>, 6); else go(model_kernel<3, true, true>, 7); }
    }
}

}
```

bert.cpp_amd/csrc/options.cpp:

```cpp
#include "options.h"

#include <cstdio>
#include <cstdlib>

#include "weights.h"

namespace bert_hip {

#ifdef BERT_HIP_TEST_ROUTES
static constexpr bool TEST_ROUTES = true;
#else
static constexpr bool TEST_ROUTES = false;
#endif

int EngineOptions::pool_mode() const { return (pool_cls ? POOL_CLS : 0) | (normalize ? 0 : POOL_RAW); }

void EngineOptions::apply(const std::string &key, const std::string &value) {
    const int n = atoi(value.c_str());
    if (key == "pooling" || key == "normalize") {
        const bool pooling = key == "pooling";
        const char *const on = pooling ? "cls" : "1", *const off = pooling ? "mean" : "0";
        if (value == on || value == off) (pooling ? pool_cls : normalize) = value == on;
        else fprintf(stderr, "bert_hip: %s = \"%s\": expected \"%s\" or \"%s\"; ignored\n", key.c_str(), value.c_str(), off, on);
        return;
    }
    if (key == "gemm") gemm_naive = value == "naive";
    else if (key == "attn") attn_naive = value == "naive";
    else if (key == "qkv2") qkv2 = value != "0";
    else if (key == "gemm256") gemm256 = value != "0";
    else if (key == "ln_fold") ln_fold = value != "0";
    else if (key == "tail") tail = value != "0";
    else if (key == "latency") latency = value != "0";
    else if (key == "stage_kernel") stage_kernel = value != "0";
    else if (key == "window_slots") set_window_slots(n);
    else if (key == "latency_tokens") { if (n >= 32) latency_tokens = n; }
    else if (key == "one_launch") one_launch = value == "0" ? 0 : value == "2" ? 2 : 1;
    else if (key == "f32") f32_exact = value != "f16";
    else if (key == "chunk_tokens") { if (n > 0) chunk_tokens = n; }
}

EngineOptions EngineOptions::from_env(const HParams &hp) {
    EngineOptions o;
    if (hp.n_embd < 256) o.latency_tokens = 128;
    const std::string kernels = getenv("BERT_HIP_KERNELS") ? getenv("BERT_HIP_KERNELS") : "";
    if (kernels == "naive" && TEST_ROUTES) o.gemm_naive = o.attn_naive = true;
    else if (kernels == "naive") fprintf(stderr, "BERT_HIP_KERNELS=naive: a test cross-check (libbert_test.so), not a route of libbert.so; ignored\n");
    else if (kernels == "tiled") o.qkv2 = o.tail = o.latency = false, o.one_launch = 0;
    if (const char *v = getenv("BERT_HIP_Q4")) o.q4_expand = std::string(v) != "fused";
    static const char *const same_as_key[][2] = {
        {"BERT_HIP_LATENCY", "latency"}, {"BERT_HIP_LATENCY", "latency_tokens"},
        {"BERT_HIP_LN_FOLD", "ln_fold"},
        {"BERT_HIP_CHUNK_TOKENS", "chunk_tokens"}, {"BERT_HIP_WINDOW_SLOTS", "window_slots"},
        {"BERT_HIP_F32", "f32"},
        {"BERT_HIP_POOLING", "pooling"}, {"BERT_HIP_NORMALIZE", "normalize"},
    };
    for (auto &ek : same_as_key)
        if (const char *v = getenv(ek[0])) o.apply(ek[1], v);
    return o;
}

void EngineOptions::set(const std::string &key, const std::string &value, bool naive_images, bool fold_images) {
    if (!TEST_ROUTES && (key == "gemm" || key == "attn") && value == "naive")
        fprintf(stderr, "bert_hip_set_option: %s=naive is a test cross-check (libbert_test.so), not a route of libbert.so; ignored\n", key.c_str());
    else if (key == "gemm" && value == "naive" && !naive_images)
        fprintf(stderr, "bert_hip_set_option: gemm=naive needs BERT_HIP_KERNELS=naive at load time (the f16 row-major images were not built); ignored\n");
    else if (key == "ln_fold" && value != "0" && !fold_images)
        fprintf(stderr, "bert_hip_set_option: ln_fold=1 needs BERT_HIP_LN_FOLD=1 at load time (the folded images were not built); ignored\n");
    else apply(key, value);
}

bool test_poison_option(const std::string &key, const DevBuf &ctx) {
    if (!TEST_ROUTES || key != "test_poison_ctx") return false;
    (void)hipDeviceSynchronize();
    if (ctx.p) (void)hipMemset(ctx.p, 0xFF, ctx.bytes);
    (void)hipDeviceSynchronize();
    return true;
}

}
```

bert.cpp_amd/csrc/options.h:

```cpp
#pragma once
#include <string>

#include "model_file.h"

namespace bert_hip {

struct DevBuf;

struct EngineOptions {
    bool gemm_naive = false, attn_naive = false;
    bool qkv2 = true, gemm256 = true, tail = true;
    bool ln_fold = true;
    bool latency = true;
    bool q4_expand = true;
    bool f32_exact = true;
    int one_launch = 1;
    int chunk_tokens = 262144;
    int latency_tokens = 768;
    bool stage_kernel = true;
    bool pool_cls = false, normalize = true;
    int pool_mode() const;

    static EngineOptions from_env(const HParams &hp);
    void set(const std::string &key, const std::string &value, bool naive_images, bool fold_images);

private:
    void apply(const std::string &key, const std::string &value);
};

bool test_poison_option(const std::string &key, const DevBuf &ctx);

}
```

bert.cpp_amd/csrc/profiler.h:

```cpp
#pragma once
#include <hip/hip_runtime.h>

#include <map>
#include <string>
#include <vector>

#include "kernels.h"

namespace bert_hip {

class LaunchProfiler {
public:
    LaunchProfiler() = default;
    LaunchProfiler(const LaunchProfiler &) = delete;
    LaunchProfiler &operator=(const LaunchProfiler &) = delete;
    ~LaunchProfiler();

    void enable(bool on) { profiling_ = on; }
    void set_replay(const std::string &value);
    void begin_pass() { replay_done_ = false; }
    void count_family(const std::string &family) { if (profiling_ && replay_name_.empty()) families_[family] += 1; }
    template <class F> void timed(const char *name, double flops, hipStream_t s, F &&f) {
        if (!profiling_) f();
        else if (!replay_name_.empty()) replay(name, flops, s, f);
        else {
            Pending p{name, get_event(), get_event(), flops, 1};
            LaunchTiming lt{p.a, p.b, 0};
            tl_launch_timing = &lt;
            f();
            tl_launch_timing = nullptr;
            if (lt.launches == 1) pending_.push_back(p);
            else { ev_pool_.push_back(p.a); ev_pool_.push_back(p.b); }
        }
    }
    std::string report();

private:
    struct Pending { const char *name; hipEvent_t a, b; double flops; int launches; };
    struct KernelStat { int launches = 0; double ms = 0.0; double flops = 0.0; };
    hipEvent_t get_event();
    template <class F> void replay(const char *name, double flops, hipStream_t s, F &&f) {
        f();
        if (replay_done_ || replay_name_ != name) return;
        replay_done_ = true;
        warn_replay();
        Pending p{name, get_event(), get_event(), flops * replay_k_, replay_k_};
        (void)hipEventRecord(p.a, s);
        for (int k = 0; k < replay_k_; ++k) f();
        (void)hipEventRecord(p.b, s);
        pending_.push_back(p);
    }
    static void warn_replay();

    bool profiling_ = false;
    std::vector<hipEvent_t> ev_pool_;
    std::string replay_name_;
    int replay_k_ = 10;
    bool replay_done_ = false;
    std::vector<Pending> pending_;
    std::map<std::string, KernelStat> stats_;
    std::map<std::string, int> families_;
};

}
```

bert.cpp_amd/pybert.py:

```python
from __future__ import annotations

import ctypes as C
import os
import subprocess
from typing import List, Optional, Sequence

import numpy as np

_HERE = os.path.dirname(os.path.abspath(__file__))
LIB_PATH = os.environ.get("BERT_HIP_LIB") or os.path.join(_HERE, "libbert.so")

BERT_H_SYMBOLS = [
    "bert_params_parse", "bert_load_from_file", "bert_free", "bert_encode", "bert_encode_batch", "bert_tokenize",
    "bert_eval", "bert_eval_batch", "bert_n_embd", "bert_n_max_tokens", "bert_vocab_id_to_token",
]
BERT_HIP_H_SYMBOLS = [
    "bert_hip_load_tokenizer", "bert_hip_tokenize_batch", "bert_hip_n_layer", "bert_hip_n_head", "bert_hip_n_intermediate", "bert_hip_n_vocab",
    "bert_hip_ftype", "bert_hip_device", "bert_hip_n_devices", "bert_hip_pooling", "bert_hip_normalize", "bert_hip_encode_batch", "bert_hip_eval_packed", "bert_hip_eval_packed_gather",
    "bert_hip_eval_packed_device", "bert_hip_reserve", "bert_hip_check", "bert_hip_eval_hidden",
    "bert_hip_profile_enable", "bert_hip_profile_report", "bert_hip_set_option", "bert_hip_version",
    "bert_hip_index_create", "bert_hip_index_free", "bert_hip_index_size", "bert_hip_index_reserve", "bert_hip_index_add",
    "bert_hip_index_add_device", "bert_hip_index_add_texts", "bert_hip_index_search", "bert_hip_index_search_device",
    "bert_hip_index_search_texts", "bert_hip_index_remove", "bert_hip_index_n_live", "bert_hip_index_search_filtered",
    "bert_hip_index_search_filtered_device", "bert_hip_index_compact", "bert_hip_index_save", "bert_hip_index_load",
    "bert_hip_index_rescore", "bert_hip_index_rescore_device", "bert_hip_index_search_rescored", "bert_hip_index_search_rescored_device",
    "bert_hip_index_get_rows", "bert_hip_index_partition", "bert_hip_index_n_lists", "bert_hip_index_partition_centroids",
    "bert_hip_index_partition_lists", "bert_hip_index_kmeans", "bert_hip_index_search_probed", "bert_hip_index_search_probed_device",
]
BERT_HIP_TEST_H_SYMBOLS = [
    "bert_hip_test_gemm", "bert_hip_test_gemm_lnfold", "bert_hip_test_attention", "bert_hip_test_qkv_attention",
    "bert_hip_test_layer_tail", "bert_hip_test_shard_bounds", "bert_hip_test_build_windows",
    "bert_hip_test_build_windows_device", "bert_hip_test_max_windows", "bert_hip_test_set_window_slots",
    "bert_hip_test_dispatch", "bert_hip_test_shard_threads_created", "bert_hip_test_embed_ln", "bert_hip_test_pool_normalize",
    "bert_hip_test_pool",
    "bert_hip_test_model_digest", "bert_hip_test_pack_weight", "bert_hip_test_parse_devices", "bert_hip_test_gather_runs",
    "bert_hip_test_encode_groups", "bert_hip_test_tokenize_pack", "bert_hip_test_index_header",
    "bert_hip_test_build_lists",
]
TEST_LIB_PATH = LIB_PATH[:-3] + "_test.so"


def build(force: bool = False, jobs: int = 8) -> str:
    args = ["make", "-C", _HERE, f"-j{jobs}", "-s"]
    if force:
        args.append("-B")
    subprocess.check_call(args)
    return LIB_PATH


_lib = None


def _declare_product_abi(L):
    vp, i32, f32p, i32p = C.c_void_p, C.c_int32, C.POINTER(C.c_float), C.POINTER(C.c_int32)
    L.bert_load_from_file.restype = vp; L.bert_load_from_file.argtypes = [C.c_char_p]
    L.bert_hip_load_tokenizer.restype = vp; L.bert_hip_load_tokenizer.argtypes = [C.c_char_p]
    L.bert_free.restype = None; L.bert_free.argtypes = [vp]
    for fn in ("bert_n_embd", "bert_n_max_tokens", "bert_hip_n_layer", "bert_hip_n_head", "bert_hip_n_intermediate",
               "bert_hip_n_vocab", "bert_hip_ftype", "bert_hip_device", "bert_hip_pooling", "bert_hip_normalize"):
        getattr(L, fn).restype = i32; getattr(L, fn).argtypes = [vp]
    L.bert_vocab_id_to_token.restype = C.c_char_p; L.bert_vocab_id_to_token.argtypes = [vp, i32]
    L.bert_tokenize.restype = None; L.bert_tokenize.argtypes = [vp, C.c_char_p, i32p, i32p, i32]
    L.bert_eval.restype = None; L.bert_eval.argtypes = [vp, i32, i32p, i32, f32p]
    L.bert_eval_batch.restype = None
    L.bert_eval_batch.argtypes = [vp, i32, i32, C.POINTER(i32p), i32p, C.POINTER(f32p)]
    L.bert_encode.restype = None; L.bert_encode.argtypes = [vp, i32, C.c_char_p, f32p]
    L.bert_encode_batch.restype = None
    L.bert_encode_batch.argtypes = [vp, i32, i32, i32, C.POINTER(C.c_char_p), C.POINTER(f32p)]
    L.bert_hip_eval_packed.restype = i32; L.bert_hip_eval_packed.argtypes = [vp, i32p, i32p, i32, f32p]
    L.bert_hip_eval_packed_device.restype = i32
    L.bert_hip_eval_packed_device.argtypes = [vp, vp, vp, i32, i32, i32, vp, vp]
    L.bert_hip_eval_hidden.restype = i32; L.bert_hip_eval_hidden.argtypes = [vp, i32p, i32, f32p, f32p]
    L.bert_hip_profile_enable.restype = None; L.bert_hip_profile_enable.argtypes = [vp, i32]
    L.bert_hip_profile_report.restype = i32; L.bert_hip_profile_report.argtypes = [vp, C.c_char_p, i32]
    L.bert_hip_set_option.restype = None; L.bert_hip_set_option.argtypes = [vp, C.c_char_p, C.c_char_p]
    L.bert_hip_n_devices.restype = i32; L.bert_hip_n_devices.argtypes = [vp]
    L.bert_hip_encode_batch.restype = i32
    L.bert_hip_encode_batch.argtypes = [vp, i32, i32, C.POINTER(C.c_char_p), C.POINTER(f32p)]
    L.bert_hip_eval_packed_gather.restype = i32
    L.bert_hip_eval_packed_gather.argtypes = [vp, i32p, i32p, i32, C.POINTER(vp)]
    L.bert_hip_reserve.restype = i32; L.bert_hip_reserve.argtypes = [vp, i32, i32]
    L.bert_hip_check.restype = i32; L.bert_hip_check.argtypes = [vp]
    L.bert_hip_tokenize_batch.restype = i32
    L.bert_hip_tokenize_batch.argtypes = [vp, i32, i32, C.POINTER(C.c_char_p), i32p, i32p]
    L.bert_hip_version.restype = C.c_char_p
    L.bert_hip_index_create.restype = vp; L.bert_hip_index_create.argtypes = [vp, i32, i32]
    L.bert_hip_index_free.restype = None; L.bert_hip_index_free.argtypes = [vp]
    L.bert_hip_index_size.restype = i32; L.bert_hip_index_size.argtypes = [vp]
    L.bert_hip_index_reserve.restype = i32; L.bert_hip_index_reserve.argtypes = [vp, i32, i32, i32]
    L.bert_hip_index_add.restype = i32; L.bert_hip_index_add.argtypes = [vp, i32, f32p]
    L.bert_hip_index_add_device.restype = i32; L.bert_hip_index_add_device.argtypes = [vp, i32, vp, vp]
    L.bert_hip_index_add_texts.restype = i32; L.bert_hip_index_add_texts.argtypes = [vp, i32, i32, C.POINTER(C.c_char_p)]
    L.bert_hip_index_search.restype = i32; L.bert_hip_index_search.argtypes = [vp, i32, f32p, i32, i32p, f32p]
    L.bert_hip_index_search_device.restype = i32; L.bert_hip_index_search_device.argtypes = [vp, i32, vp, i32, vp, vp, vp]
    L.bert_hip_index_search_texts.restype = i32
    L.bert_hip_index_search_texts.argtypes = [vp, i32, i32, C.POINTER(C.c_char_p), i32, i32p, f32p]
    L.bert_hip_index_remove.restype = i32; L.bert_hip_index_remove.argtypes = [vp, i32, i32p]
    L.bert_hip_index_n_live.restype = i32; L.bert_hip_index_n_live.argtypes = [vp]
    L.bert_hip_index_search_filtered.restype = i32; L.bert_hip_index_search_filtered.argtypes = [vp, i32, f32p, i32, vp, i32, i32p, f32p]
    L.bert_hip_index_search_filtered_device.restype = i32
    L.bert_hip_index_search_filtered_device.argtypes = [vp, i32, vp, i32, vp, i32, vp, vp, vp]
    L.bert_hip_index_compact.restype = i32; L.bert_hip_index_compact.argtypes = [vp, i32p]
    L.bert_hip_index_save.restype = i32; L.bert_hip_index_save.argtypes = [vp, C.c_char_p]
    L.bert_hip_index_load.restype = vp; L.bert_hip_index_load.argtypes = [vp, C.c_char_p]
    L.bert_hip_index_rescore.restype = i32; L.bert_hip_index_rescore.argtypes = [vp, i32, f32p, i32, i32p, i32, i32p, f32p]
    L.bert_hip_index_rescore_device.restype = i32; L.bert_hip_index_rescore_device.argtypes = [vp, i32, vp, i32, vp, i32, vp, vp, vp]
    L.bert_hip_index_search_rescored.restype = i32; L.bert_hip_index_search_rescored.argtypes = [vp, vp, i32, f32p, i32, i32, i32p, f32p]
    L.bert_hip_index_search_rescored_device.restype = i32
    L.bert_hip_index_search_rescored_device.argtypes = [vp, vp, i32, vp, i32, i32, vp, vp, vp]
    L.bert_hip_index_get_rows.restype = i32; L.bert_hip_index_get_rows.argtypes = [vp, i32, i32p, f32p]
    L.bert_hip_index_partition.restype = i32; L.bert_hip_index_partition.argtypes = [vp, i32, f32p]
    L.bert_hip_index_n_lists.restype = i32; L.bert_hip_index_n_lists.argtypes = [vp]
    L.bert_hip_index_partition_centroids.restype = i32; L.bert_hip_index_partition_centroids.argtypes = [vp, f32p]
    L.bert_hip_index_partition_lists.restype = i32; L.bert_hip_index_partition_lists.argtypes = [vp, i32p]
    L.bert_hip_index_kmeans.restype = i32; L.bert_hip_index_kmeans.argtypes = [vp, i32, i32, f32p]
    L.bert_hip_index_search_probed.restype = i32; L.bert_hip_index_search_probed.argtypes = [vp, i32, f32p, i32, i32, i32p, f32p]
    L.bert_hip_index_search_probed_device.restype = i32; L.bert_hip_index_search_probed_device.argtypes = [vp, i32, vp, i32, i32, vp, vp, vp]


def lib() -> C.CDLL:
    global _lib
    if _lib is not None:
        return _lib
    if not os.path.exists(LIB_PATH):
        raise RuntimeError(f"{LIB_PATH} not found: build the HIP extension first "
                           f"(python -c 'import __graft_entry__ as g; g.build()' or make -C bert.cpp_amd)")
    L = C.CDLL(LIB_PATH)
    _declare_product_abi(L)
    _lib = L
    return L


_test_lib = None


def test_lib() -> C.CDLL:
    global _test_lib
    if _test_lib is not None:
        return _test_lib
    if not os.path.exists(TEST_LIB_PATH):
        raise RuntimeError(f"{TEST_LIB_PATH} not found: build it first (make -C bert.cpp_amd)")
    L = C.CDLL(TEST_LIB_PATH)
    _declare_product_abi(L)
    vp, i32, i32p = C.c_void_p, C.c_int32, C.POINTER(C.c_int32)
    L.bert_hip_test_gemm.restype = i32
    L.bert_hip_test_gemm.argtypes = [i32, i32, i32, vp, vp, i32, vp, vp, i32, i32, vp]
    L.bert_hip_test_gemm_lnfold.restype = i32
    L.bert_hip_test_gemm_lnfold.argtypes = [i32, i32, i32, i32] + [vp] * 10 + [i32, vp, vp, vp]
    L.bert_hip_test_attention.restype = i32
    L.bert_hip_test_attention.argtypes = [i32, i32p, i32, i32, vp, i32, vp]
    L.bert_hip_test_qkv_attention.restype = i32
    L.bert_hip_test_qkv_attention.argtypes = [i32, i32p, i32, i32, vp, vp, i32, vp, i32, vp]
    L.bert_hip_test_layer_tail.restype = i32
    L.bert_hip_test_layer_tail.argtypes = [i32, i32, i32, vp, vp, vp, vp, vp, i32, vp, vp, vp, vp, vp, vp, vp, i32, vp]
    L.bert_hip_test_embed_ln.restype = i32
    L.bert_hip_test_embed_ln.argtypes = [i32, i32, i32, i32, vp, vp, vp, vp, vp, i32p, i32p, i32, vp]
    L.bert_hip_test_pool_normalize.restype = i32
    L.bert_hip_test_pool_normalize.argtypes = [i32, vp, i32p, i32, i32, vp, i32p]
    L.bert_hip_test_pool.restype = i32
    L.bert_hip_test_pool.argtypes = [i32, vp, i32p, i32, i32, i32, i32, vp, i32p]
    L.bert_hip_test_model_digest.restype = i32
    L.bert_hip_test_model_digest.argtypes = [C.c_char_p, i32p, C.POINTER(C.c_uint64)]
    L.bert_hip_test_pack_weight.restype = i32
    L.bert_hip_test_pack_weight.argtypes = [vp, i32, i32, i32, i32, vp, vp, vp, vp, C.c_int64]
    L.bert_hip_test_shard_bounds.restype = None
    L.bert_hip_test_shard_bounds.argtypes = [i32p, i32, i32, i32p]
    L.bert_hip_test_build_windows.restype = i32
    L.bert_hip_test_build_windows.argtypes = [i32p, i32, i32p]
    L.bert_hip_test_max_windows.restype = i32
    L.bert_hip_test_max_windows.argtypes = [i32, i32]
    L.bert_hip_test_set_window_slots.restype = i32
    L.bert_hip_test_set_window_slots.argtypes = [i32]
    L.bert_hip_test_build_windows_device.restype = i32
    L.bert_hip_test_build_windows_device.argtypes = [i32p, i32, i32p]
    L.bert_hip_test_shard_threads_created.restype = C.c_int64
    L.bert_hip_test_shard_threads_created.argtypes = []
    L.bert_hip_test_dispatch.restype = i32
    L.bert_hip_test_dispatch.argtypes = [i32p, i32p, i32, i32, i32, C.POINTER(C.c_float)]
    L.bert_hip_test_parse_devices.restype = i32
    L.bert_hip_test_parse_devices.argtypes = [C.c_char_p, i32, i32, i32p, C.c_char_p, i32]
    L.bert_hip_test_gather_runs.restype = i32
    L.bert_hip_test_gather_runs.argtypes = [i32p, i32, C.c_int64, i32p]
    L.bert_hip_test_encode_groups.restype = i32
    L.bert_hip_test_encode_groups.argtypes = [i32, i32p, i32]
    L.bert_hip_test_tokenize_pack.restype = i32
    L.bert_hip_test_tokenize_pack.argtypes = [vp, i32, i32, C.POINTER(C.c_char_p), i32p, i32p, i32p, i32p, i32]
    L.bert_hip_test_index_header.restype = i32
    L.bert_hip_test_index_header.argtypes = [C.c_char_p, i32, C.c_int64, C.POINTER(C.c_uint32), C.c_char_p, i32]
    L.bert_hip_test_build_lists.restype = i32
    L.bert_hip_test_build_lists.argtypes = [i32p, i32, i32, i32p, i32p]
    _test_lib = L
    return L


def test_embed_ln(table_type: int, word_bytes, type_bytes, pos_bytes, H: int, gamma, beta, tokens, cu_seqlens) -> np.ndarray:
    wb, tb, pb = (np.ascontiguousarray(a) for a in (word_bytes, type_bytes, pos_bytes))
    rb = {0: 4 * H, 1: 2 * H, 2: H // 32 * 18, 3: H // 32 * 20}[table_type]
    g = np.ascontiguousarray(gamma, dtype=np.float32); b = np.ascontiguousarray(beta, dtype=np.float32)
    toks = np.ascontiguousarray(tokens, dtype=np.int32); cu = np.ascontiguousarray(cu_seqlens, dtype=np.int32)
    out = np.zeros((len(toks), H), dtype=np.float16)
    r = test_lib().bert_hip_test_embed_ln(table_type, H, wb.nbytes // rb, pb.nbytes // rb, wb.ctypes.data, tb.ctypes.data, pb.ctypes.data,
                                          g.ctypes.data, b.ctypes.data, _i32p(toks), _i32p(cu), len(cu) - 1, out.ctypes.data)
    if r != 0:
        raise RuntimeError(f"bert_hip_test_embed_ln failed: {r}")
    return out


def test_pool_normalize(x: np.ndarray, cu_seqlens, max_len: int):
    x = np.ascontiguousarray(x, dtype=np.float16); cu = np.ascontiguousarray(cu_seqlens, dtype=np.int32)
    out = np.zeros((len(cu) - 1, x.shape[1]), dtype=np.float32)
    st = np.zeros(1, dtype=np.int32)
    r = test_lib().bert_hip_test_pool_normalize(x.shape[1], x.ctypes.data, _i32p(cu), len(cu) - 1, max_len, out.ctypes.data, _i32p(st))
    if r != 0:
        raise RuntimeError(f"bert_hip_test_pool_normalize failed: {r}")
    return out, int(st[0])


def test_pool(x: np.ndarray, cu_seqlens, max_len: int, pooling: str = "mean", normalize: bool = True):
    x = np.ascontiguousarray(x, dtype=np.float16); cu = np.ascontiguousarray(cu_seqlens, dtype=np.int32)
    out = np.zeros((len(cu) - 1, x.shape[1]), dtype=np.float32)
    st = np.zeros(1, dtype=np.int32)
    r = test_lib().bert_hip_test_pool(x.shape[1], x.ctypes.data, _i32p(cu), len(cu) - 1, max_len, {"mean": 0, "cls": 1}[pooling],
                                      int(bool(normalize)), out.ctypes.data, _i32p(st))
    if r != 0:
        raise RuntimeError(f"bert_hip_test_pool failed: {r}")
    return out, int(st[0])


def model_digest(path: str):
    leg = C.c_int32(0)
    dig = C.c_uint64(0)
    n = test_lib().bert_hip_test_model_digest(path.encode(), C.byref(leg), C.byref(dig))
    if n < 0:
        raise RuntimeError("model file rejected (see stderr)")
    return n, bool(leg.value), int(dig.value)


PACK_FORMS = {"f16": 0, "f16_kperm": 1, "q4_nibbles": 2, "q4_scales": 3, "ln_fold": 4, "ln_fold_stats": 5, "gamma_beta_bias": 6, "table_f32": 7}


def pack_weight(W, wtype: int, N: int, K: int, form: str, gamma=None, beta=None, bias=None, stack3: bool = False) -> np.ndarray:
    Wb = np.ascontiguousarray(W)
    f32 = [None if a is None else np.ascontiguousarray(a, dtype=np.float32) for a in (gamma, beta, bias)]
    out = np.zeros((N + 127) // 128 * 128 * max(K, 16) * 4, dtype=np.uint8)
    n = test_lib().bert_hip_test_pack_weight(Wb.ctypes.data, wtype, N, K, PACK_FORMS[form] | (0x100 if stack3 else 0),
                                             *(None if a is None else a.ctypes.data for a in f32), out.ctypes.data, out.nbytes)
    if n < 0:
        raise RuntimeError(f"bert_hip_test_pack_weight failed: {n}")
    return out[:n].copy()


def shard_bounds(cu_seqlens: np.ndarray, n_shards: int) -> List[int]:
    cu = np.ascontiguousarray(cu_seqlens, dtype=np.int32)
    out = np.zeros(n_shards + 1, dtype=np.int32)
    test_lib().bert_hip_test_shard_bounds(_i32p(cu), len(cu) - 1, n_shards, _i32p(out))
    return out.tolist()


def build_windows(cu_seqlens: np.ndarray, device: bool = False) -> List[tuple]:
    cu = np.ascontiguousarray(cu_seqlens, dtype=np.int32)
    out = np.zeros(2 * max(len(cu) - 1, 1), dtype=np.int32)
    f = test_lib().bert_hip_test_build_windows_device if device else test_lib().bert_hip_test_build_windows
    n = f(_i32p(cu), len(cu) - 1, _i32p(out))
    if n < 0:
        raise RuntimeError("bert_hip_test_build_windows_device failed")
    return [(int(out[2 * i]), int(out[2 * i + 1])) for i in range(n)]


def set_window_slots(slots: int) -> int:
    return int(test_lib().bert_hip_test_set_window_slots(slots))


def max_windows(n_sentences: int, n_tokens: int) -> int:
    return int(test_lib().bert_hip_test_max_windows(n_sentences, n_tokens))


def dispatch_stub(tokens: np.ndarray, cu_seqlens: np.ndarray, n_shards: int, H: int = 4, throw: bool = False) -> np.ndarray:
    tokens = np.ascontiguousarray(tokens, dtype=np.int32)
    cu = np.ascontiguousarray(cu_seqlens, dtype=np.int32)
    out = np.full((len(cu) - 1, abs(H)), np.nan, dtype=np.float32)
    r = test_lib().bert_hip_test_dispatch(_i32p(tokens), _i32p(cu), len(cu) - 1, n_shards, -H if throw else H, _f32p(out))
    if r != 0:
        raise RuntimeError(f"bert_hip_test_dispatch failed: {r}")
    return out


def shard_threads_created() -> int:
    return int(test_lib().bert_hip_test_shard_threads_created())


def parse_devices(spec: Optional[bytes], n_devices: int, current: int = 0):
    devs = np.zeros(max(n_devices, 1), dtype=np.int32)
    err = C.create_string_buffer(512)
    n = test_lib().bert_hip_test_parse_devices(spec, n_devices, current, _i32p(devs), err, len(err))
    return (None, err.value.decode()) if n < 0 else (devs[:n].tolist(), None)


def gather_runs(cu_seqlens: np.ndarray, tokens_per_run: int) -> List[int]:
    cu = np.ascontiguousarray(cu_seqlens, dtype=np.int32)
    out = np.zeros(len(cu), dtype=np.int32)
    n = test_lib().bert_hip_test_gather_runs(_i32p(cu), len(cu) - 1, tokens_per_run, _i32p(out))
    return out[:n].tolist()


def encode_groups(n_inputs: int) -> List[int]:
    out = np.zeros(1024, dtype=np.int32)
    n = test_lib().bert_hip_test_encode_groups(n_inputs, _i32p(out), len(out))
    assert n <= len(out)
    return out[:n].tolist()


def tokenize_pack(model: "BertModel", texts: Sequence[bytes], n_threads: int, counts=None):
    n, N = len(texts), model.n_max_tokens
    arr = (C.c_char_p * n)(*texts)
    cnt = np.zeros(n, dtype=np.int32)
    cu = np.full(n + 1, -1, dtype=np.int32)
    packed = np.full(n * N, -1, dtype=np.int32)
    given = None if counts is None else np.ascontiguousarray(counts, dtype=np.int32)
    n_ok = test_lib().bert_hip_test_tokenize_pack(model.ctx, n_threads, n, arr, None if given is None else _i32p(given), _i32p(cnt),
                                                  _i32p(cu), _i32p(packed), len(packed))
    if n_ok < 0:
        raise RuntimeError("bert_hip_test_tokenize_pack failed")
    return n_ok, cnt.tolist(), cu[:n_ok + 1].tolist(), packed[:cu[n_ok]].tolist()


def _f32p(a: np.ndarray):
    return a.ctypes.data_as(C.POINTER(C.c_float))


def _i32p(a: np.ndarray):
    return a.ctypes.data_as(C.POINTER(C.c_int32))


class BertModel:

    def __init__(self, fname: str, tokenizer_only: bool = False, test_routes: bool = False):
        self.lib = test_lib() if test_routes else lib()
        load = self.lib.bert_hip_load_tokenizer if tokenizer_only else self.lib.bert_load_from_file
        self.ctx = load(fname.encode("utf-8"))
        if not self.ctx:
            raise RuntimeError(f"bert_load_from_file('{fname}') failed (see stderr)")
        self.n_embd = self.lib.bert_n_embd(self.ctx)
        self.n_max_tokens = self.lib.bert_n_max_tokens(self.ctx)
        self.n_layer = self.lib.bert_hip_n_layer(self.ctx)
        self.n_vocab = self.lib.bert_hip_n_vocab(self.ctx)

    def close(self):
        if getattr(self, "ctx", None):
            self.lib.bert_free(self.ctx)
            self.ctx = None

    def __del__(self):
        try:
            self.close()
        except Exception:
            pass

    def tokenize(self, text: str | bytes, n_max_tokens: Optional[int] = None) -> List[int]:
        n_max = n_max_tokens or self.n_max_tokens
        buf = (C.c_int32 * max(n_max, 2))()
        n = C.c_int32(0)
        data = text if isinstance(text, bytes) else text.encode("utf-8")
        self.lib.bert_tokenize(self.ctx, data, buf, C.byref(n), n_max)
        return list(buf[: n.value])

    def tokenize_batch(self, texts: Sequence[str | bytes], n_threads: int = 6) -> List[List[int]]:
        n, N = len(texts), self.n_max_tokens
        arr = (C.c_char_p * n)(*[t if isinstance(t, bytes) else t.encode("utf-8") for t in texts])
        toks = np.zeros((n, N), dtype=np.int32)
        cnt = np.zeros(n, dtype=np.int32)
        if self.lib.bert_hip_tokenize_batch(self.ctx, n_threads, n, arr, _i32p(toks), _i32p(cnt)) != 0:
            raise RuntimeError("bert_hip_tokenize_batch failed")
        return [toks[i, : cnt[i]].tolist() for i in range(n)]

    def id_to_token(self, i: int) -> bytes:
        return self.lib.bert_vocab_id_to_token(self.ctx, i)

    def eval(self, tokens: Sequence[int], n_threads: int = 6) -> np.ndarray:
        toks = np.ascontiguousarray(tokens, dtype=np.int32)
        out = np.full(self.n_embd, np.nan, dtype=np.float32)
        self.lib.bert_eval(self.ctx, n_threads, _i32p(toks), len(toks), _f32p(out))
        return out

    def eval_batch(self, sentences: Sequence[Sequence[int]], n_threads: int = 6, scattered: bool = False) -> np.ndarray:
        B = len(sentences)
        arrs = [np.ascontiguousarray(s, dtype=np.int32) for s in sentences]
        wide = np.full((B, 2 * self.n_embd + 3 if scattered else self.n_embd), np.nan, dtype=np.float32)
        out = wide[:, : self.n_embd]
        tok_ptrs = (C.POINTER(C.c_int32) * B)(*[_i32p(a) for a in arrs])
        lens = np.array([len(a) for a in arrs], dtype=np.int32)
        out_ptrs = (C.POINTER(C.c_float) * B)(*[C.cast(wide[i].ctypes.data, C.POINTER(C.c_float)) for i in range(B)])
        self.lib.bert_eval_batch(self.ctx, n_threads, B, tok_ptrs, _i32p(lens), out_ptrs)
        if scattered:
            assert np.isnan(wide[:, self.n_embd:]).all()
        return np.ascontiguousarray(out)

    def encode(self, text: str, n_threads: int = 6) -> np.ndarray:
        out = np.full(self.n_embd, np.nan, dtype=np.float32)
        self.lib.bert_encode(self.ctx, n_threads, text.encode("utf-8"), _f32p(out))
        return out

    def encode_batch(self, texts: Sequence[str], n_threads: int = 6, batch_size: int = 16) -> np.ndarray:
        n = len(texts)
        out = np.full((n, self.n_embd), np.nan, dtype=np.float32)
        out_ptrs = (C.POINTER(C.c_float) * n)(*[_f32p(out[i]) for i in range(n)])
        txt = (C.c_char_p * n)(*[t.encode("utf-8") for t in texts])
        self.lib.bert_encode_batch(self.ctx, n_threads, batch_size, n, txt, out_ptrs)
        return out

    def eval_packed(self, tokens: np.ndarray, cu_seqlens: np.ndarray, out: Optional[np.ndarray] = None) -> np.ndarray:
        tokens = np.ascontiguousarray(tokens, dtype=np.int32)
        cu = np.ascontiguousarray(cu_seqlens, dtype=np.int32)
        B = len(cu) - 1
        if out is None:
            out = np.full((B, self.n_embd), np.nan, dtype=np.float32)
        assert out.dtype == np.float32 and out.flags.c_contiguous and out.shape == (B, self.n_embd)
        r = self.lib.bert_hip_eval_packed(self.ctx, _i32p(tokens), _i32p(cu), B, _f32p(out))
        if r != 0:
            raise RuntimeError(f"bert_hip_eval_packed failed: {r}")
        return out

    def n_devices(self) -> int:
        return self.lib.bert_hip_n_devices(self.ctx)

    def eval_packed_gather(self, tokens: np.ndarray, cu_seqlens: np.ndarray) -> List[int]:
        tokens = np.ascontiguousarray(tokens, dtype=np.int32)
        cu = np.ascontiguousarray(cu_seqlens, dtype=np.int32)
        ptrs = (C.c_void_p * self.n_devices())()
        r = self.lib.bert_hip_eval_packed_gather(self.ctx, _i32p(tokens), _i32p(cu), len(cu) - 1, ptrs)
        if r != 0:
            raise RuntimeError(f"bert_hip_eval_packed_gather failed: {r}")
        return [int(p) for p in ptrs]

    def reserve(self, n_tokens: int, n_sentences: int) -> None:
        if self.lib.bert_hip_reserve(self.ctx, n_tokens, n_sentences) != 0:
            raise RuntimeError("bert_hip_reserve failed")

    def check(self) -> int:
        return self.lib.bert_hip_check(self.ctx)

    def encode_batch_count(self, texts: Sequence[str], n_threads: int = 6):
        n = len(texts)
        out = np.full((n, self.n_embd), np.nan, dtype=np.float32)
        out_ptrs = (C.POINTER(C.c_float) * n)(*[_f32p(out[i]) for i in range(n)])
        txt = (C.c_char_p * n)(*[t.encode("utf-8") for t in texts])
        return self.lib.bert_hip_encode_batch(self.ctx, n_threads, n, txt, out_ptrs), out

    def eval_packed_device(self, d_tokens_ptr: int, d_cu_ptr: int, n_sentences: int, n_tokens: int, max_len: int,
                           d_out_ptr: int, stream: int = 0) -> None:
        r = self.lib.bert_hip_eval_packed_device(self.ctx, d_tokens_ptr, d_cu_ptr, n_sentences, n_tokens, max_len,
                                                 d_out_ptr, stream)
        if r != 0:
            raise RuntimeError(f"bert_hip_eval_packed_device failed: {r}")

    def eval_hidden(self, tokens: Sequence[int]):
        toks = np.ascontiguousarray(tokens, dtype=np.int32)
        hid = np.empty((self.n_layer + 1, len(toks), self.n_embd), dtype=np.float32)
        out = np.empty(self.n_embd, dtype=np.float32)
        r = self.lib.bert_hip_eval_hidden(self.ctx, _i32p(toks), len(toks), _f32p(hid), _f32p(out))
        if r != 0:
            raise RuntimeError(f"bert_hip_eval_hidden failed: {r}")
        return out, hid

    def profile(self, on: bool) -> None:
        self.lib.bert_hip_profile_enable(self.ctx, int(on))

    def profile_report(self, families: bool = False) -> dict:
        buf = C.create_string_buffer(1 << 16)
        self.lib.bert_hip_profile_report(self.ctx, buf, len(buf))
        out = {}
        for line in buf.value.decode().splitlines():
            name, launches, ms, flops = line.split()
            if families or not name.startswith("family:"):
                out[name] = {"launches": int(launches), "total_ms": float(ms), "flops_per_launch": float(flops)}
        return out

    def set_option(self, key: str, value: str) -> None:
        self.lib.bert_hip_set_option(self.ctx, key.encode(), value.encode())

    def pooling(self) -> int:
        return int(self.lib.bert_hip_pooling(self.ctx))

    def normalize(self) -> int:
        return int(self.lib.bert_hip_normalize(self.ctx))

    def index(self, dim: Optional[int] = None, dtype: str = "f16") -> "BertIndex":
        return BertIndex(self, dim, dtype)

    def load_index(self, path: str) -> "BertIndex":
        return BertIndex(self, _load=path)


def allow_words(allow, n_rows: int) -> np.ndarray:
    a = np.asarray(allow)
    if a.dtype == np.uint32:
        return np.ascontiguousarray(a).reshape(-1)
    if a.dtype != np.bool_ or a.shape != (n_rows,):
        raise ValueError(f"allow must be a bool array of {n_rows} entries or uint32 words")
    packed = np.packbits(a, bitorder="little").tobytes().ljust((n_rows + 31) // 32 * 4, b"\0")
    return np.frombuffer(packed, dtype="<u4").astype(np.uint32)


class BertIndex:

    def __init__(self, model: BertModel, dim: Optional[int] = None, dtype: str = "f16", _load: Optional[str] = None):
        if dtype not in ("f16", "f32", "i8", "b1"):
            raise ValueError("dtype must be 'f16', 'f32', 'i8' or 'b1'")
        self.model, self.lib = model, model.lib
        if _load is not None:
            self.ix = self.lib.bert_hip_index_load(model.ctx, os.fsencode(_load))
            if not self.ix:
                raise RuntimeError("bert_hip_index_load failed (see stderr)")
            with open(_load, "rb") as f:
                head = np.frombuffer(f.read(24), dtype="<u4")
            self.dtype, self.dim = ("f32", "f16", "i8", "b1")[int(head[3])], int(head[4])
            return
        code = {"f16": 1, "i8": 2, "b1": 3}.get(dtype, 0)
        self.ix = self.lib.bert_hip_index_create(model.ctx, 0 if dim is None else int(dim), code)
        if not self.ix:
            raise RuntimeError("bert_hip_index_create failed (see stderr)")
        self.dim = model.n_embd if dim is None else int(dim)
        self.dtype = dtype

    def close(self):
        if getattr(self, "ix", None) and getattr(self.model, "ctx", None):
            self.lib.bert_hip_index_free(self.ix)
        self.ix = None

    def __del__(self):
        try:
            self.close()
        except Exception:
            pass

    def __len__(self) -> int:
        return int(self.lib.bert_hip_index_size(self.ix))

    def reserve(self, n_rows: int, n_queries: int = 0, k: int = 1) -> None:
        if self.lib.bert_hip_index_reserve(self.ix, n_rows, n_queries, k) != 0:
            raise RuntimeError("bert_hip_index_reserve failed")

    def add(self, rows) -> int:
        rows = np.ascontiguousarray(rows, dtype=np.float32).reshape(-1, self.dim)
        r = self.lib.bert_hip_index_add(self.ix, rows.shape[0], _f32p(rows))
        if r < 0:
            raise RuntimeError(f"bert_hip_index_add failed: {r}")
        return r

    def add_device(self, n: int, d_rows_ptr: int, stream: int = 0) -> int:
        r = self.lib.bert_hip_index_add_device(self.ix, n, d_rows_ptr, stream)
        if r < 0:
            raise RuntimeError(f"bert_hip_index_add_device failed: {r}")
        return r

    def add_texts(self, texts: Sequence[str], n_threads: int = 6) -> int:
        n = len(texts)
        txt = (C.c_char_p * n)(*[t.encode("utf-8") for t in texts])
        r = self.lib.bert_hip_index_add_texts(self.ix, n_threads, n, txt)
        if r < 0:
            raise RuntimeError(f"bert_hip_index_add_texts failed: {r}")
        return r

    def search(self, queries, k: int = 10, allow=None):
        q = np.ascontiguousarray(queries, dtype=np.float32).reshape(-1, self.dim)
        ids = np.empty((q.shape[0], k), dtype=np.int32)
        scores = np.empty((q.shape[0], k), dtype=np.float32)
        if allow is None:
            r = self.lib.bert_hip_index_search(self.ix, q.shape[0], _f32p(q), k, _i32p(ids), _f32p(scores))
            if r != 0:
                raise RuntimeError(f"bert_hip_index_search failed: {r}")
            return ids, scores
        words = allow_words(allow, len(self))
        r = self.lib.bert_hip_index_search_filtered(self.ix, q.shape[0], _f32p(q), k, words.ctypes.data, len(words), _i32p(ids), _f32p(scores))
        if r != 0:
            raise RuntimeError(f"bert_hip_index_search_filtered failed: {r}")
        return ids, scores

    def search_device(self, n_queries: int, d_queries_ptr: int, k: int, d_ids_ptr: int, d_scores_ptr: int, stream: int = 0,
                      d_allow_ptr: Optional[int] = None, n_words: int = 0) -> None:
        if d_allow_ptr is None:
            r = self.lib.bert_hip_index_search_device(self.ix, n_queries, d_queries_ptr, k, d_ids_ptr, d_scores_ptr, stream)
            if r != 0:
                raise RuntimeError(f"bert_hip_index_search_device failed: {r}")
            return
        r = self.lib.bert_hip_index_search_filtered_device(self.ix, n_queries, d_queries_ptr, k, d_allow_ptr, n_words, d_ids_ptr, d_scores_ptr, stream)
        if r != 0:
            raise RuntimeError(f"bert_hip_index_search_filtered_device failed: {r}")

    def rescore(self, queries, cand_ids, k: int = 10):
        q = np.ascontiguousarray(queries, dtype=np.float32).reshape(-1, self.dim)
        cand = np.ascontiguousarray(cand_ids, dtype=np.int32).reshape(q.shape[0], -1)
        ids = np.empty((q.shape[0], k), dtype=np.int32)
        scores = np.empty((q.shape[0], k), dtype=np.float32)
        r = self.lib.bert_hip_index_rescore(self.ix, q.shape[0], _f32p(q), cand.shape[1], _i32p(cand), k, _i32p(ids), _f32p(scores))
        if r != 0:
            raise RuntimeError(f"bert_hip_index_rescore failed: {r}")
        return ids, scores

    def rescore_device(self, n_queries: int, d_queries_ptr: int, n_cand: int, d_cand_ptr: int, k: int, d_ids_ptr: int,
                       d_scores_ptr: int, stream: int = 0) -> None:
        r = self.lib.bert_hip_index_rescore_device(self.ix, n_queries, d_queries_ptr, n_cand, d_cand_ptr, k, d_ids_ptr, d_scores_ptr, stream)
        if r != 0:
            raise RuntimeError(f"bert_hip_index_rescore_device failed: {r}")

    def search_rescored(self, fine: "BertIndex", queries, k: int = 10, n_cand: int = 100):
        q = np.ascontiguousarray(queries, dtype=np.float32).reshape(-1, self.dim)
        ids = np.empty((q.shape[0], k), dtype=np.int32)
        scores = np.empty((q.shape[0], k), dtype=np.float32)
        r = self.lib.bert_hip_index_search_rescored(self.ix, fine.ix, q.shape[0], _f32p(q), n_cand, k, _i32p(ids), _f32p(scores))
        if r != 0:
            raise RuntimeError(f"bert_hip_index_search_rescored failed: {r}")
        return ids, scores

    def search_rescored_device(self, fine: "BertIndex", n_queries: int, d_queries_ptr: int, n_cand: int, k: int, d_ids_ptr: int,
                               d_scores_ptr: int, stream: int = 0) -> None:
        r = self.lib.bert_hip_index_search_rescored_device(self.ix, fine.ix, n_queries, d_queries_ptr, n_cand, k, d_ids_ptr, d_scores_ptr, stream)
        if r != 0:
            raise RuntimeError(f"bert_hip_index_search_rescored_device failed: {r}")

    def get_rows(self, ids) -> np.ndarray:
        ids = np.ascontiguousarray(ids, dtype=np.int32).reshape(-1)
        rows = np.empty((len(ids), self.dim), dtype=np.float32)
        r = self.lib.bert_hip_index_get_rows(self.ix, len(ids), _i32p(ids), _f32p(rows))
        if r != 0:
            raise RuntimeError(f"bert_hip_index_get_rows failed: {r}")
        return rows

    def kmeans(self, n_lists: int, n_iter: int, centroids) -> np.ndarray:
        c = np.array(centroids, dtype=np.float32, order="C").reshape(n_lists, self.dim)
        r = self.lib.bert_hip_index_kmeans(self.ix, n_lists, n_iter, _f32p(c))
        if r != 0:
            raise RuntimeError(f"bert_hip_index_kmeans failed: {r}")
        return c

    def partition(self, centroids) -> None:
        c = np.zeros((0, self.dim), np.float32) if centroids is None else np.ascontiguousarray(centroids, dtype=np.float32).reshape(-1, self.dim)
        r = self.lib.bert_hip_index_partition(self.ix, c.shape[0], _f32p(c))
        if r != 0:
            raise RuntimeError(f"bert_hip_index_partition failed: {r}")

    @property
    def n_lists(self) -> int:
        return int(self.lib.bert_hip_index_n_lists(self.ix))

    def centroids(self) -> np.ndarray:
        c = np.empty((max(self.n_lists, 0), self.dim), dtype=np.float32)
        r = self.lib.bert_hip_index_partition_centroids(self.ix, _f32p(c))
        if r != 0:
            raise RuntimeError(f"bert_hip_index_partition_centroids failed: {r}")
        return c

    def partition_lists(self) -> np.ndarray:
        lists = np.empty(len(self), dtype=np.int32)
        r = self.lib.bert_hip_index_partition_lists(self.ix, _i32p(lists))
        if r != 0:
            raise RuntimeError(f"bert_hip_index_partition_lists failed: {r}")
        return lists

    def live_ids(self) -> np.ndarray:
        n = len(self)
        if self.n_live == n:
            return np.arange(n, dtype=np.int32)
        cand = np.full((n + 255) // 256 * 256, -1, np.int32)
        cand[:n] = np.arange(n, dtype=np.int32)
        ids, _ = self.rescore(np.zeros((len(cand) // 256, self.dim), np.float32), cand.reshape(-1, 256), 256)
        return np.sort(ids[ids >= 0])

    def train_partition(self, n_lists: int, n_iter: int = 10, seed: int = 0) -> np.ndarray:
        pick = np.random.default_rng(seed).choice(self.live_ids(), n_lists, replace=False)
        c = self.kmeans(n_lists, n_iter, self.get_rows(pick))
        self.partition(c)
        return c

    def search_probed(self, queries, k: int = 10, nprobe: int = 8):
        q = np.ascontiguousarray(queries, dtype=np.float32).reshape(-1, self.dim)
        ids = np.empty((q.shape[0], k), dtype=np.int32)
        scores = np.empty((q.shape[0], k), dtype=np.float32)
        r = self.lib.bert_hip_index_search_probed(self.ix, q.shape[0], _f32p(q), nprobe, k, _i32p(ids), _f32p(scores))
        if r != 0:
            raise RuntimeError(f"bert_hip_index_search_probed failed: {r}")
        return ids, scores

    def search_probed_device(self, n_queries: int, d_queries_ptr: int, nprobe: int, k: int, d_ids_ptr: int, d_scores_ptr: int,
                             stream: int = 0) -> None:
        r = self.lib.bert_hip_index_search_probed_device(self.ix, n_queries, d_queries_ptr, nprobe, k, d_ids_ptr, d_scores_ptr, stream)
        if r != 0:
            raise RuntimeError(f"bert_hip_index_search_probed_device failed: {r}")

    @property
    def n_live(self) -> int:
        return int(self.lib.bert_hip_index_n_live(self.ix))

    def remove(self, ids) -> int:
        ids = np.ascontiguousarray(ids, dtype=np.int32).reshape(-1)
        r = self.lib.bert_hip_index_remove(self.ix, len(ids), _i32p(ids))
        if r < 0:
            raise RuntimeError(f"bert_hip_index_remove failed: {r}")
        return r

    def compact(self) -> np.ndarray:
        old = np.empty(max(self.n_live, 0), dtype=np.int32)
        r = self.lib.bert_hip_index_compact(self.ix, _i32p(old))
        if r < 0:
            raise RuntimeError(f"bert_hip_index_compact failed: {r}")
        return old[:r]

    def save(self, path: str) -> None:
        r = self.lib.bert_hip_index_save(self.ix, os.fsencode(path))
        if r != 0:
            raise RuntimeError(f"bert_hip_index_save failed: {r}")

    def search_texts(self, texts: Sequence[str], k: int = 10, n_threads: int = 6):
        n = len(texts)
        txt = (C.c_char_p * max(n, 1))(*[t.encode("utf-8") for t in texts])
        ids = np.empty((n, k), dtype=np.int32)
        scores = np.empty((n, k), dtype=np.float32)
        r = self.lib.bert_hip_index_search_texts(self.ix, n_threads, n, txt, k, _i32p(ids), _f32p(scores))
        if r != 0:
            raise RuntimeError(f"bert_hip_index_search_texts failed: {r}")
        return ids, scores


def test_gemm(A: np.ndarray, W_bytes: np.ndarray, wtype: int, N: int, bias: np.ndarray,
              resid: Optional[np.ndarray], epilogue: int, impl: int) -> np.ndarray:
    L = test_lib()
    A = np.ascontiguousarray(A, dtype=np.float16)
    M, K = A.shape
    Wb = np.ascontiguousarray(W_bytes)
    bias = np.ascontiguousarray(bias, dtype=np.float32)
    out = np.zeros((M, N), dtype=np.float16)
    rp = None
    if resid is not None:
        resid = np.ascontiguousarray(resid, dtype=np.float16)
        rp = resid.ctypes.data
    r = L.bert_hip_test_gemm(M, N, K, A.ctypes.data, Wb.ctypes.data, wtype, bias.ctypes.data, rp, epilogue, impl,
                             out.ctypes.data)
    if r != 0:
        raise RuntimeError(f"bert_hip_test_gemm failed: {r}")
    return out


def test_gemm_lnfold(A1, W1, b1, r, rg, rb, W2, b2, g, be, epi2):
    L = test_lib()
    A1 = np.ascontiguousarray(A1, dtype=np.float16); W1 = np.ascontiguousarray(W1, dtype=np.float16); W2 = np.ascontiguousarray(W2, dtype=np.float16)
    r = np.ascontiguousarray(r, dtype=np.float16)
    f = lambda v: None if v is None else np.ascontiguousarray(v, dtype=np.float32)
    b1, rg, rb, b2, g, be = f(b1), f(rg), f(rb), f(b2), f(g), f(be)
    M, K1 = A1.shape
    H, N2 = W1.shape[0], W2.shape[0]
    u = np.zeros((M, H), dtype=np.float16); out = np.zeros((M, N2), dtype=np.float16); rows = np.zeros((M, 4), dtype=np.float32)
    p = lambda v: None if v is None else v.ctypes.data
    rc = L.bert_hip_test_gemm_lnfold(M, K1, H, N2, p(A1), p(W1), p(b1), p(r), p(rg), p(rb), p(W2), p(b2), p(g), p(be), epi2, p(u), p(out), p(rows))
    if rc != 0:
        raise RuntimeError(f"bert_hip_test_gemm_lnfold failed: {rc}")
    return u, out, rows


def test_attention(qkv: np.ndarray, cu_seqlens: np.ndarray, n_head: int, d_head: int, impl: int) -> np.ndarray:
    L = test_lib()
    qkv = np.ascontiguousarray(qkv, dtype=np.float16)
    cu = np.ascontiguousarray(cu_seqlens, dtype=np.int32)
    T = qkv.shape[0]
    out = np.zeros((T, n_head * d_head), dtype=np.float16)
    r = L.bert_hip_test_attention(len(cu) - 1, _i32p(cu), n_head, d_head, qkv.ctypes.data, impl, out.ctypes.data)
    if r != 0:
        raise RuntimeError(f"bert_hip_test_attention failed: {r}")
    return out


def test_qkv_attention(x: np.ndarray, cu_seqlens: np.ndarray, n_head: int, d_head: int, W_bytes: np.ndarray, wtype: int,
                       bias: np.ndarray, fused: bool) -> np.ndarray:
    L = test_lib()
    x = np.ascontiguousarray(x, dtype=np.float16)
    cu = np.ascontiguousarray(cu_seqlens, dtype=np.int32)
    w = np.ascontiguousarray(W_bytes)
    bias = np.ascontiguousarray(bias, dtype=np.float32)
    out = np.zeros((x.shape[0], n_head * d_head), dtype=np.float16)
    r = L.bert_hip_test_qkv_attention(len(cu) - 1, _i32p(cu), n_head, d_head, x.ctypes.data, w.ctypes.data, wtype,
                                      bias.ctypes.data, int(fused), out.ctypes.data)
    if r != 0:
        raise RuntimeError(f"bert_hip_test_qkv_attention failed: {r}")
    return out


def test_layer_tail(ctx: np.ndarray, x: np.ndarray, Wo_bytes, W1_bytes, W2_bytes, wtype: int, I: int, bo, g1, be1, b1, b2,
                    g2, be2, impl: int) -> np.ndarray:
    L = test_lib()
    ctx = np.ascontiguousarray(ctx, dtype=np.float16)
    x = np.ascontiguousarray(x, dtype=np.float16)
    M, H = ctx.shape
    ws = [np.ascontiguousarray(w) for w in (Wo_bytes, W1_bytes, W2_bytes)]
    f = lambda a: np.ascontiguousarray(a, dtype=np.float32)
    ps = [f(v) for v in (bo, g1, be1, b1, b2, g2, be2)]
    out = np.zeros((M, H), dtype=np.float16)
    r = L.bert_hip_test_layer_tail(M, H, I, ctx.ctypes.data, x.ctypes.data, ws[0].ctypes.data, ws[1].ctypes.data,
                                   ws[2].ctypes.data, wtype, *[p.ctypes.data for p in ps], impl, out.ctypes.data)
    if r != 0:
        raise RuntimeError(f"bert_hip_test_layer_tail failed: {r}")
    return out
```

Before: 344,900 sentences/s.

## Fold embedding layernorm into the persistent one-launch model kernel

Adds an embed-fold path in which waves 4-7 of each workgroup gather word/type/position embeddings, apply layernorm and keep the resulting fragments in registers. These feed directly into the first layer's QKV/attention phase, so the separate embed_ln kernel launch and its re-read of x are skipped. The path is used only for the one-launch route with full 128-token windows and f16 tables, and the f16 embed path now uses contract-off float arithmetic with explicit rounding. This adds register pressure and front-loaded latency to the model kernel in exchange for one less launch and one less pass over activations.

```diff
diff --git a/bert.cpp_amd/csrc/device.h b/bert.cpp_amd/csrc/device.h
--- a/bert.cpp_amd/csrc/device.h
+++ b/bert.cpp_amd/csrc/device.h
@@ -218,6 +218,99 @@
     nmr = -mean * rstd;
 }
 
+template <int TT>
+__device__ __forceinline__ void table_run8(const void *tab, int H, int r, int e0, float (&v)[8]) {
+    if (TT == 0) {
+        const float4 a = *(const float4 *)((const float *)tab + (size_t)r * H + e0);
+        const float4 b = *(const float4 *)((const float *)tab + (size_t)r * H + e0 + 4);
+        v[0] = a.x; v[1] = a.y; v[2] = a.z; v[3] = a.w; v[4] = b.x; v[5] = b.y; v[6] = b.z; v[7] = b.w;
+    } else if (TT == 1) {
+        const f16x8 h = *(const f16x8 *)((const half_t *)tab + (size_t)r * H + e0);
+#pragma unroll
+        for (int i = 0; i < 8; ++i) v[i] = (float)h[i];
+    } else {
+        constexpr int bs = TT == 2 ? 18 : 20, qo = TT == 2 ? 2 : 4;
+        const unsigned char *blk = (const unsigned char *)tab + ((size_t)r * (H / 32) + (e0 >> 5)) * bs;
+        const int off = e0 & 31;
+        const float d = (float)*(const half_t *)blk;
+        const float m = TT == 3 ? (float)*(const half_t *)(blk + 2) : 0.f;
+        unsigned short q16[4];
+#pragma unroll
+        for (int i = 0; i < 4; ++i) q16[i] = *(const unsigned short *)(blk + qo + (off & 15) + 2 * i);
+#pragma unroll
+        for (int i = 0; i < 8; ++i) {
+            const int byte = (q16[i >> 1] >> (8 * (i & 1))) & 0xff, q = off < 16 ? (byte & 0x0F) : (byte >> 4);
+            v[i] = TT == 2 ? (float)(q - 8) * d : (float)q * d + m;
+        }
+    }
+}
+template <int TT>
+__device__ __forceinline__ void embed_run8(const void *word, const void *type, const void *pos, int H, int id, int p, int e0, float (&v)[8], float &sum) {
+    float w[8], ty[8], ps[8];
+    table_run8<TT>(word, H, id, e0, w);
+    table_run8<TT>(type, H, 0, e0, ty);
+    table_run8<TT>(pos, H, p, e0, ps);
+#pragma unroll
+    for (int i = 0; i < 8; ++i) { v[i] = ps[i] + (ty[i] + w[i]); sum += v[i]; }
+}
+__device__ __forceinline__ float embed_ln_mean(float total, int H) { return total / H; }
+__device__ __forceinline__ void embed_center8(float (&v)[8], float mean, float &sq) {
+#pragma clang fp contract(off)
+#pragma unroll
+    for (int i = 0; i < 8; ++i) { v[i] -= mean; sq += v[i] * v[i]; }
+}
+__device__ __forceinline__ float embed_ln_rstd(float total_sq, int H) {
+#pragma clang fp contract(off)
+    return 1.0f / sqrtf(total_sq / H + 1e-5f);
+}
+__device__ __forceinline__ f16x8 embed_out8(const float (&v)[8], float rstd, const float *__restrict__ gamma, const float *__restrict__ beta, int e0) {
+#pragma clang fp contract(off)
+    const float4 g0 = *(const float4 *)(gamma + e0), g1 = *(const float4 *)(gamma + e0 + 4);
+    const float4 b0 = *(const float4 *)(beta + e0), b1 = *(const float4 *)(beta + e0 + 4);
+    const float gg[8] = {g0.x, g0.y, g0.z, g0.w, g1.x, g1.y, g1.z, g1.w};
+    const float bb[8] = {b0.x, b0.y, b0.z, b0.w, b1.x, b1.y, b1.z, b1.w};
+    f16x8 o;
+#pragma unroll
+    for (int i = 0; i < 8; ++i) o[i] = (_Float16)rounded_f32(__builtin_fmaf(gg[i], v[i] * rstd, bb[i]));
+    return o;
+}
+template <int NQ>
+__device__ __forceinline__ float embed_lane_tree_sum(const float (&s)[NQ]) {
+    static_assert(NQ > 0 && NQ <= 32, "half a row of at most 512 features");
+    float zero = 0.f;
+    asm volatile("" : "+v"(zero));
+    float a[32];
+#pragma unroll
+    for (int q = 0; q < 32; ++q) a[q] = q < NQ ? s[q] : zero;
+#pragma unroll
+    for (int step = 16; step >= 1; step >>= 1)
+#pragma unroll
+        for (int q = 0; q < step; ++q) a[q] = a[q] + a[q + step];
+    return xor32_sum(a[0]);
+}
+template <int NQ, int TT>
+__device__ __forceinline__ void embed_ln_fragments(const void *word, const void *type, const void *pos, const float *__restrict__ gamma,
+                                                   const float *__restrict__ beta, const int32_t *__restrict__ tokens, int n_vocab, int window,
+                                                   int blk, int lane, half_t *__restrict__ x, f16x8 (&xf)[NQ]) {
+    constexpr int H = 16 * NQ;
+    const int l31 = lane & 31, hi = lane >> 5, p = 32 * blk + l31;
+    const size_t t = (size_t)window * 128 + p;
+    int id = tokens[t];
+    id = id < 0 ? 0 : (id >= n_vocab ? n_vocab - 1 : id);
+    float v[NQ][8], s[NQ];
+#pragma unroll
+    for (int q = 0; q < NQ; ++q) { s[q] = 0.f; embed_run8<TT>(word, type, pos, H, id, p, 16 * q + 8 * hi, v[q], s[q]); }
+    const float mean = embed_ln_mean(embed_lane_tree_sum(s), H);
+#pragma unroll
+    for (int q = 0; q < NQ; ++q) { s[q] = 0.f; embed_center8(v[q], mean, s[q]); }
+    const float rstd = embed_ln_rstd(embed_lane_tree_sum(s), H);
+#pragma unroll
+    for (int q = 0; q < NQ; ++q) {
+        xf[q] = embed_out8(v[q], rstd, gamma, beta, 16 * q + 8 * hi);
+        *(f16x8 *)(x + t * H + 16 * q + 8 * hi) = xf[q];
+    }
+}
+
 struct RawBlock { uint4 q; unsigned sc; };
 template <int WT>
 __device__ __forceinline__ RawBlock q4_load_block(const uint4 *qs, const void *sc, size_t index) {
diff --git a/bert.cpp_amd/csrc/engine.h b/bert.cpp_amd/csrc/engine.h
--- a/bert.cpp_amd/csrc/engine.h
+++ b/bert.cpp_amd/csrc/engine.h
@@ -33,6 +33,8 @@
     int check(std::string &err);
     void set_option(const std::string &key, const std::string &value);
     void profile_enable(bool on) { prof_.enable(on); }
+    void test_poison_x();
+    bool test_last_pass_embed_fold() const { return last_embed_fold_; }
     std::string profile_report();
     void timed_launch(const char *name, double flops, hipStream_t s, const std::function<void()> &f);
 
@@ -61,6 +63,7 @@
         const int2 *windows;
         int n_windows;
         Route route = Route::LAYERED;
+        bool embed_fold = false;
         bool build_windows = false;
         const int *n_windows_dev = nullptr;
         std::vector<LayerPlan> layers;
@@ -83,6 +86,7 @@
     EngineOptions opt_;
     std::unique_ptr<ModelWeights> w_;
     LaunchProfiler prof_;
+    bool last_embed_fold_ = false;
 
     DevBuf x_, qkv_, ctx_, y_, ff_, v32_, d_tokens_, d_cu_, d_out_, d_hidden_, status_, windows_;
     DevBuf ln_stats1_, ln_stats2_, ln_rows1_, ln_rows2_;
diff --git a/bert.cpp_amd/csrc/engine.hip b/bert.cpp_amd/csrc/engine.hip
--- a/bert.cpp_amd/csrc/engine.hip
+++ b/bert.cpp_amd/csrc/engine.hip
@@ -79,6 +79,13 @@
            windows_.ensure((size_t)n_sentences * sizeof(int2), err) &&
            (!(H > 384 && H % 256 == 0) || (ln_stats1_.ensure(tp * (2 * H / 256) * 8, err) && ln_stats2_.ensure(tp * (2 * H / 256) * 8, err) &&
                                            ln_rows1_.ensure(tp * 16, err) && ln_rows2_.ensure(tp * 16, err)));
+}
+
+void Engine::test_poison_x() {
+    (void)hipSetDevice(device_);
+    (void)hipDeviceSynchronize();
+    if (x_.p) (void)hipMemset(x_.p, 0xFF, x_.bytes);
+    (void)hipDeviceSynchronize();
 }
 
 void Engine::timed_launch(const char *name, double flops, hipStream_t s, const std::function<void()> &f) { timed(name, flops, s, f); }
@@ -115,9 +122,11 @@
     HIP_OK(hipStreamWaitEvent(s, busy_, 0), err, -1);
     const Plan p = plan(d_tokens, d_cu, B, T, max_len, d_out, s, d_hidden, d_windows, n_windows, slots, pool_mode);
     bool ok = true;
+    last_embed_fold_ = p.embed_fold;
     if (p.route == Route::F32) ok = forward_f32(p, err);
     else {
         const int H = hp_.n_embd;
+        if (!p.embed_fold)
         timed("embed_ln", 0.0, s, [&] { launch_embed_ln(w_->word_emb.p, w_->type_emb.p, w_->pos_emb.p, w_->table_type, w_->ln_e_w.as<float>(), w_->ln_e_b.as<float>(),
                                                         d_tokens, d_cu, B, T, H, hp_.n_vocab, max_len, x_.as<half_t>(), s); });
         tap(p, 0);
@@ -181,6 +190,8 @@
     const bool skinny = latency_call && opt_.tail && opt_.qkv2 && !opt_.gemm_naive && !opt_.attn_naive && max_len <= 128 && (dh == 32 || dh == 64) &&
                         skinny_layer_supported(L0.qkv.w, L0.o.w, L0.ffi.w, L0.ffo.w) && qkv2_shape0;
     p.route = skinny ? Route::LATENCY : one_launch && one_launch_pays ? Route::ONE_LAUNCH : fold ? Route::FOLDED : Route::LAYERED;
+    p.embed_fold = p.route == Route::ONE_LAUNCH && full_windows && opt_.embed_fold && w_->table_type == 1 && hp_.n_max_tokens >= 128 &&
+                   !d_hidden && !prof_.enabled();
     return p;
 }
 
@@ -250,9 +261,10 @@
         mw[il] = {&L.qkv.w, &L.o.w, &L.ffi.w, &L.ffo.w, L.qkv_b.as<float>(), L.o_b.as<float>(), L.ln_att_w.as<float>(), L.ln_att_b.as<float>(),
                   L.ffi_b.as<float>(), L.ffo_b.as<float>(), L.ln_out_w.as<float>(), L.ln_out_b.as<float>()};
     }
+    const ModelEmbedding emb = {p.tokens, w_->word_emb.p, w_->type_emb.p, w_->pos_emb.p, w_->table_type, hp_.n_vocab, w_->ln_e_w.as<float>(), w_->ln_e_b.as<float>()};
     timed("model_kernel", hp_.n_layer * (2.0 * p.T * 3 * H * H + 4.0 * p.T * p.max_len * H + 2.0 * p.T * H * H + 4.0 * p.T * H * I), p.s, [&] {
         launch_model_kernel(mw, hp_.n_layer, x_.as<half_t>(), ctx_.as<half_t>(), p.cu, p.B, p.T, p.windows, p.n_windows, p.n_windows_dev, hp_.n_head,
-                            p.out, p.max_len, status_.as<int>(), p.pool_mode, p.slots, p.s);
+                            p.out, p.max_len, status_.as<int>(), p.pool_mode, p.slots, p.s, p.embed_fold ? &emb : nullptr);
     });
 }
 
diff --git a/bert.cpp_amd/csrc/kernels.h b/bert.cpp_amd/csrc/kernels.h
--- a/bert.cpp_amd/csrc/kernels.h
+++ b/bert.cpp_amd/csrc/kernels.h
@@ -54,9 +54,15 @@
 };
 bool model_kernel_supported(const GemmWeight &Wqkv, const GemmWeight &Wo, const GemmWeight &W1, const GemmWeight &W2, int n_layer,
                             int n_head, int d_head, int max_len);
+struct ModelEmbedding {
+    const int32_t *tokens;
+    const void *word, *type, *pos;
+    int table_type, n_vocab;
+    const float *gamma, *beta;
+};
 void launch_model_kernel(const ModelLayerWeights *layers, int n_layer, half_t *x, half_t *ctx, const int32_t *cu_seqlens, int n_sentences,
                          int n_tokens, const int2 *groups, int n_groups, const int *n_groups_dev, int n_head, float *pooled, int max_len,
-                         int *status, int pool_mode, int slots, hipStream_t stream);
+                         int *status, int pool_mode, int slots, hipStream_t stream, const ModelEmbedding *embed = nullptr);
 bool skinny_layer_supported(const GemmWeight &Wqkv, const GemmWeight &Wo, const GemmWeight &W1, const GemmWeight &W2);
 void launch_skinny_gemm(int mode, const GemmWeight &W, const half_t *A, const float *V, const float *gamma, const float *beta,
                         half_t *ln_out, const float *bias, const half_t *resid, half_t *out16, float *out32, int n_token_blocks,
diff --git a/bert.cpp_amd/csrc/misc_kernels.hip b/bert.cpp_amd/csrc/misc_kernels.hip
--- a/bert.cpp_amd/csrc/misc_kernels.hip
+++ b/bert.cpp_amd/csrc/misc_kernels.hip
@@ -88,32 +88,6 @@
     }
 }
 
-template <int TT>
-__device__ __forceinline__ void table_run8(const void *tab, int H, int r, int e0, float (&v)[8]) {
-    if (TT == 0) {
-        const float4 a = *(const float4 *)((const float *)tab + (size_t)r * H + e0);
-        const float4 b = *(const float4 *)((const float *)tab + (size_t)r * H + e0 + 4);
-        v[0] = a.x; v[1] = a.y; v[2] = a.z; v[3] = a.w; v[4] = b.x; v[5] = b.y; v[6] = b.z; v[7] = b.w;
-    } else if (TT == 1) {
-        const f16x8 h = *(const f16x8 *)((const half_t *)tab + (size_t)r * H + e0);
-#pragma unroll
-        for (int i = 0; i < 8; ++i) v[i] = (float)h[i];
-    } else {
-        constexpr int bs = TT == 2 ? 18 : 20, qo = TT == 2 ? 2 : 4;
-        const unsigned char *blk = (const unsigned char *)tab + ((size_t)r * (H / 32) + (e0 >> 5)) * bs;
-        const int off = e0 & 31;
-        const float d = (float)*(const half_t *)blk;
-        const float m = TT == 3 ? (float)*(const half_t *)(blk + 2) : 0.f;
-        unsigned short q16[4];
-#pragma unroll
-        for (int i = 0; i < 4; ++i) q16[i] = *(const unsigned short *)(blk + qo + (off & 15) + 2 * i);
-#pragma unroll
-        for (int i = 0; i < 8; ++i) {
-            const int byte = (q16[i >> 1] >> (8 * (i & 1))) & 0xff, q = off < 16 ? (byte & 0x0F) : (byte >> 4);
-            v[i] = TT == 2 ? (float)(q - 8) * d : (float)q * d + m;
-        }
-    }
-}
 template <int TT, int NC, bool SEARCH>
 __global__ __launch_bounds__(256) void embed_ln_rows_kernel(const void *word, const void *type, const void *pos,
                                                             const float *__restrict__ gamma, const float *__restrict__ beta,
@@ -140,42 +114,65 @@
     }
     int id = tokens[t];
     id = id < 0 ? 0 : (id >= n_vocab ? n_vocab - 1 : id);
-    float v[NC][8];
-    float sum = 0.f;
-#pragma unroll
-    for (int j = 0; j < NC; ++j) {
-        const int e0 = 8 * (lane + 64 * j);
-#pragma unroll
-        for (int i = 0; i < 8; ++i) v[j][i] = 0.f;
-        if (e0 < H) {
-            float w[8], ty[8], ps[8];
-            table_run8<TT>(word, H, id, e0, w);
-            table_run8<TT>(type, H, 0, e0, ty);
-            table_run8<TT>(pos, H, p, e0, ps);
-#pragma unroll
-            for (int i = 0; i < 8; ++i) { v[j][i] = ps[i] + (ty[i] + w[i]); sum += v[j][i]; }
-        }
-    }
-    const float mean = wave_sum_f32(sum) / H;
-    float sq = 0.f;
-#pragma unroll
-    for (int j = 0; j < NC; ++j)
-        if (8 * (lane + 64 * j) < H)
-#pragma unroll
-            for (int i = 0; i < 8; ++i) { v[j][i] -= mean; sq += v[j][i] * v[j][i]; }
-    const float rstd = 1.0f / sqrtf(wave_sum_f32(sq) / H + 1e-5f);
-#pragma unroll
-    for (int j = 0; j < NC; ++j) {
-        const int e0 = 8 * (lane + 64 * j);
-        if (e0 < H) {
-            const float4 g0 = *(const float4 *)(gamma + e0), g1 = *(const float4 *)(gamma + e0 + 4);
-            const float4 b0 = *(const float4 *)(beta + e0), b1 = *(const float4 *)(beta + e0 + 4);
-            const float gg[8] = {g0.x, g0.y, g0.z, g0.w, g1.x, g1.y, g1.z, g1.w};
-            const float bb[8] = {b0.x, b0.y, b0.z, b0.w, b1.x, b1.y, b1.z, b1.w};
-            f16x8 o;
-#pragma unroll
-            for (int i = 0; i < 8; ++i) o[i] = (_Float16)(gg[i] * (v[j][i] * rstd) + bb[i]);
-            *(f16x8 *)(out + (size_t)t * H + e0) = o;
+    if constexpr (TT <= 1) {
+        float v[NC][8];
+        float sum = 0.f;
+#pragma unroll
+        for (int j = 0; j < NC; ++j) {
+            const int e0 = 8 * (lane + 64 * j);
+#pragma unroll
+            for (int i = 0; i < 8; ++i) v[j][i] = 0.f;
+            if (e0 < H) embed_run8<TT>(word, type, pos, H, id, p, e0, v[j], sum);
+        }
+        const float mean = embed_ln_mean(wave_sum_f32(sum), H);
+        float sq = 0.f;
+#pragma unroll
+        for (int j = 0; j < NC; ++j)
+            if (8 * (lane + 64 * j) < H) embed_center8(v[j], mean, sq);
+        const float rstd = embed_ln_rstd(wave_sum_f32(sq), H);
+#pragma unroll
+        for (int j = 0; j < NC; ++j) {
+            const int e0 = 8 * (lane + 64 * j);
+            if (e0 < H) *(f16x8 *)(out + (size_t)t * H + e0) = embed_out8(v[j], rstd, gamma, beta, e0);
+        }
+    } else {
+        float v[NC][8];
+        float sum = 0.f;
+#pragma unroll
+        for (int j = 0; j < NC; ++j) {
+            const int e0 = 8 * (lane + 64 * j);
+#pragma unroll
+            for (int i = 0; i < 8; ++i) v[j][i] = 0.f;
+            if (e0 < H) {
+                float w[8], ty[8], ps[8];
+                table_run8<TT>(word, H, id, e0, w);
+                table_run8<TT>(type, H, 0, e0, ty);
+                table_run8<TT>(pos, H, p, e0, ps);
+#pragma unroll
+                for (int i = 0; i < 8; ++i) { v[j][i] = ps[i] + (ty[i] + w[i]); sum += v[j][i]; }
+            }
+        }
+        const float mean = wave_sum_f32(sum) / H;
+        float sq = 0.f;
+#pragma unroll
+        for (int j = 0; j < NC; ++j)
+            if (8 * (lane + 64 * j) < H)
+#pragma unroll
+                for (int i = 0; i < 8; ++i) { v[j][i] -= mean; sq += v[j][i] * v[j][i]; }
+        const float rstd = 1.0f / sqrtf(wave_sum_f32(sq) / H + 1e-5f);
+#pragma unroll
+        for (int j = 0; j < NC; ++j) {
+            const int e0 = 8 * (lane + 64 * j);
+            if (e0 < H) {
+                const float4 g0 = *(const float4 *)(gamma + e0), g1 = *(const float4 *)(gamma + e0 + 4);
+                const float4 b0 = *(const float4 *)(beta + e0), b1 = *(const float4 *)(beta + e0 + 4);
+                const float gg[8] = {g0.x, g0.y, g0.z, g0.w, g1.x, g1.y, g1.z, g1.w};
+                const float bb[8] = {b0.x, b0.y, b0.z, b0.w, b1.x, b1.y, b1.z, b1.w};
+                f16x8 o;
+#pragma unroll
+                for (int i = 0; i < 8; ++i) o[i] = (_Float16)(gg[i] * (v[j][i] * rstd) + bb[i]);
+                *(f16x8 *)(out + (size_t)t * H + e0) = o;
+            }
         }
     }
 }
diff --git a/bert.cpp_amd/csrc/model_kernel.hip b/bert.cpp_amd/csrc/model_kernel.hip
--- a/bert.cpp_amd/csrc/model_kernel.hip
+++ b/bert.cpp_amd/csrc/model_kernel.hip
@@ -32,91 +32,25 @@
     int max_len, pool_mode;
     ModelLayerArgs layer[MODEL_MAX_LAYERS];
 };
+struct ModelEmbedArgs : ModelArgs {
+    const int32_t *tokens;
+    const void *word, *type, *pos;
+    const float *ge, *bee;
+    int n_vocab;
+};
 
 }
 
 template <int NT, bool RAGGED, bool POOL_MODES>
 __global__ __launch_bounds__(512, 2) void model_kernel(ModelArgs m) {
-    extern __shared__ __attribute__((aligned(16))) char smem[];
-    const int window = (int)blockIdx.x;
-    int tok0 = window * 128, rows = 128, first = window, count = 1;
-    if constexpr (RAGGED) {
-        if (m.groups) {
-            if (m.n_groups && window >= *m.n_groups) return;
-            const int2 g = m.groups[window];
-            first = g.x; count = g.y;
-        }
-        if (count <= 0 || first >= m.n_sent) return;
-        tok0 = m.cu[first];
-        rows = min(m.cu[first + count] - tok0, 128);
-    }
-    const int wave_index = __builtin_amdgcn_readfirstlane((int)threadIdx.x >> 6);
-    auto thread_id = [&]() __attribute__((always_inline)) {
-        int ln = (int)__builtin_amdgcn_mbcnt_hi(~0u, __builtin_amdgcn_mbcnt_lo(~0u, 0u)), w = wave_index;
-        asm volatile("" : "+v"(ln), "+s"(w));
-        return w * 64 + ln;
-    };
-    MK_STAMP(0);
-    const int n_layer = rows > 0 ? m.n_layer : 0;
-    auto window_phase = [&](const ModelLayerArgs &L, auto xregs_tag, const f16x8 *xf, f16x8 *cf) __attribute__((always_inline)) {
-        const int tid = thread_id();
-        Qkv2Args q;
-        q.x = m.x; q.w = L.wqkv; q.qs = nullptr; q.sc = nullptr; q.bias = L.bqkv; q.cu = m.cu; q.groups = RAGGED ? m.groups : nullptr; q.n_groups = nullptr;
-        q.out = m.ctx; q.n_head = m.n_head; q.n_sent = m.n_sent; q.spw = 1; q.slot_mask = m.slot_mask;
-        qkv_attention2_body<2 * NT, NT, GW_F16, !RAGGED, decltype(xregs_tag)::value, !RAGGED>(q, smem, window, tid, xf, cf);
-    };
-    auto tail_phase = [&](const ModelLayerArgs &L, f16x8 (&xf)[8 * NT], const f16x8 *cf) __attribute__((always_inline)) {
-        const int tid = thread_id();
-        TailArgs t;
-        t.ctx = m.ctx; t.x = m.x; t.wo = L.wo; t.w1p = L.w1p; t.w2p = L.w2p;
-        t.wo_qs = t.w1_qs = t.w2_qs = nullptr; t.wo_sc = t.w1_sc = t.w2_sc = nullptr;
-        t.bo = L.bo; t.g1 = L.g1; t.be1 = L.be1; t.b1 = L.b1; t.b2 = L.b2; t.g2 = L.g2; t.be2 = L.be2; t.out = m.x; t.I = m.I;
-        layer_tail_body<NT, GW_F16, RAGGED, !RAGGED, !RAGGED>(t, smem, tok0, rows, tid, xf, cf);
-    };
-    auto hand_over = [&]() __attribute__((always_inline)) {
-        __builtin_amdgcn_fence(__ATOMIC_RELEASE, "workgroup");
-        asm volatile("s_waitcnt vmcnt(0) lgkmcnt(0)\n\ts_barrier" ::: "memory");
-        __builtin_amdgcn_fence(__ATOMIC_ACQUIRE, "workgroup");
-    };
-    if constexpr (RAGGED) {
-        for (int l = 0; l < n_layer; ++l) {
-            f16x8 none[8 * NT];
-            window_phase(m.layer[l], std::false_type{}, nullptr, nullptr);
-            hand_over();
-            MK_STAMP(1 + 2 * l);
-            tail_phase(m.layer[l], none, nullptr);
-            hand_over();
-            MK_STAMP(2 + 2 * l);
-        }
-    } else {
-        f16x8 cf[8 * NT];
-        if (n_layer > 0) window_phase(m.layer[0], std::false_type{}, nullptr, cf);
-        for (int l = 0; l < n_layer; ++l) {
-            hand_over();
-            MK_STAMP(1 + 2 * l);
-            f16x8 xf[8 * NT];
-            tail_phase(m.layer[l], xf, cf);
-            hand_over();
-            MK_STAMP(2 + 2 * l);
-            if (l + 1 < n_layer) window_phase(m.layer[l + 1], std::true_type{}, xf, cf);
-            else {
-#pragma unroll
-                for (int q = 0; q < 8 * NT; ++q) asm volatile("" : "=v"(cf[q]));
-            }
-        }
-    }
-    if (m.pooled) {
-        const int tid = thread_id();
-        for (int j = 0; j < count; ++j) {
-            const int b = first + j, t0 = m.cu[b];
-            int n = m.cu[b + 1] - t0;
-            if (!RAGGED && (t0 != tok0 || n != 128)) n = -1;
-            if constexpr (POOL_MODES) pool_normalize_sentence(m.x, t0, n, b, 128 * NT, m.max_len, m.status, m.pooled, (float *)smem, tid, tid < 256, m.pool_mode);
-            else pool_normalize_sentence<false, false>(m.x, t0, n, b, 128 * NT, m.max_len, m.status, m.pooled, (float *)smem, tid, tid < 256);
-            __syncthreads();
-        }
-    }
-    MK_STAMP(1 + 2 * n_layer);
+    constexpr int EMBED = NT * 0;
+#include "model_kernel_body.h"
+}
+template <int NT, bool POOL_MODES, int TT>
+__global__ __launch_bounds__(512, 2) void model_kernel_embed(ModelEmbedArgs m) {
+    constexpr bool RAGGED = false;
+    constexpr int EMBED = 1 + TT;
+#include "model_kernel_body.h"
 }
 
 bool model_kernel_supported(const GemmWeight &Wqkv, const GemmWeight &Wo, const GemmWeight &W1, const GemmWeight &W2, int n_layer,
@@ -128,8 +62,9 @@
 
 void launch_model_kernel(const ModelLayerWeights *layers, int n_layer, half_t *x, half_t *ctx, const int32_t *cu_seqlens, int n_sentences,
                          int n_tokens, const int2 *groups, int n_groups, const int *n_groups_dev, int n_head, float *pooled, int max_len,
-                         int *status, int pool_mode, int slots, hipStream_t stream) {
-    ModelArgs m;
+                         int *status, int pool_mode, int slots, hipStream_t stream, const ModelEmbedding *embed) {
+    ModelEmbedArgs m;
+    m.tokens = nullptr; m.word = m.type = m.pos = nullptr; m.ge = m.bee = nullptr; m.n_vocab = 0;
     m.pooled = pooled; m.status = status; m.max_len = max_len; m.pool_mode = pool_mode;
     m.x = x; m.ctx = ctx; m.cu = cu_seqlens; m.groups = groups; m.n_groups = n_groups_dev;
     m.n_layer = n_layer; m.n_head = n_head; m.n_sent = n_sentences; m.I = layers[0].W1->N; m.slot_mask = slots - 1;
@@ -145,10 +80,15 @@
     const bool full = (long long)n_sentences * 128 == n_tokens;
     if (n_head * 32 != H) { fprintf(stderr, "launch_model_kernel: n_head %d x 32 != H %d\n", n_head, H); abort(); }
     const int grid = full || !groups ? n_sentences : n_groups;
-    static DeviceFlags configured[8];
-    auto go = [&](auto kernel, int which) {
+    if (embed) {
+        if (!full || embed->table_type != 1) { fprintf(stderr, "launch_model_kernel: the embedding in the launch needs full windows and f16 tables\n"); abort(); }
+        m.tokens = embed->tokens; m.word = embed->word; m.type = embed->type; m.pos = embed->pos; m.ge = embed->gamma; m.bee = embed->beta; m.n_vocab = embed->n_vocab;
+    }
+    static DeviceFlags configured[12];
+    const ModelArgs &base = m;
+    auto go = [&](auto kernel, int which, const auto &args) {
         configure_once(configured[which], [&] { (void)hipFuncSetAttribute((const void *)kernel, hipFuncAttributeMaxDynamicSharedMemorySize, 160 * 1024); });
-        BERT_LAUNCH(kernel, dim3(grid), dim3(512), lds, stream, m);
+        BERT_LAUNCH(kernel, dim3(grid), dim3(512), lds, stream, args);
 #ifdef BERT_HIP_MODEL_TIMELINE
         static int shots = 0;
         if (grid >= 256 && shots++ == 30) {
@@ -188,12 +128,16 @@
         }
 #endif
     };
-    if (pool_mode == 0) {
-        if (full) { if (H == 256) go(model_kernel<2, false, false>, 0); else go(model_kernel<3, false, false>, 1); }
-        else { if (H == 256) go(model_kernel<2, true, false>, 2); else go(model_kernel<3, true, false>, 3); }
+    if (embed) {
+        const int which = 8 + 2 * (pool_mode != 0) + (H != 256);
+        if (pool_mode == 0) { if (H == 256) go(model_kernel_embed<2, false, 1>, which, m); else go(model_kernel_embed<3, false, 1>, which, m); }
+        else { if (H == 256) go(model_kernel_embed<2, true, 1>, which, m); else go(model_kernel_embed<3, true, 1>, which, m); }
+    } else if (pool_mode == 0) {
+        if (full) { if (H == 256) go(model_kernel<2, false, false>, 0, base); else go(model_kernel<3, false, false>, 1, base); }
+        else { if (H == 256) go(model_kernel<2, true, false>, 2, base); else go(model_kernel<3, true, false>, 3, base); }
     } else {
-        if (full) { if (H == 256) go(model_kernel<2, false, true>, 4); else go(model_kernel<3, false, true>, 5); }
-        else { if (H == 256) go(model_kernel<2, true, true>, 6); else go(model_kernel<3, true, true>, 7); }
+        if (full) { if (H == 256) go(model_kernel<2, false, true>, 4, base); else go(model_kernel<3, false, true>, 5, base); }
+        else { if (H == 256) go(model_kernel<2, true, true>, 6, base); else go(model_kernel<3, true, true>, 7, base); }
     }
 }
 
diff --git a/bert.cpp_amd/csrc/model_kernel_body.h b/bert.cpp_amd/csrc/model_kernel_body.h
--- /dev/null
+++ b/bert.cpp_amd/csrc/model_kernel_body.h
@@ -0,0 +1,95 @@
+    extern __shared__ __attribute__((aligned(16))) char smem[];
+    const int window = (int)blockIdx.x;
+    int tok0 = window * 128, rows = 128, first = window, count = 1;
+    if constexpr (RAGGED) {
+        if (m.groups) {
+            if (m.n_groups && window >= *m.n_groups) return;
+            const int2 g = m.groups[window];
+            first = g.x; count = g.y;
+        }
+        if (count <= 0 || first >= m.n_sent) return;
+        tok0 = m.cu[first];
+        rows = min(m.cu[first + count] - tok0, 128);
+    }
+    const int wave_index = __builtin_amdgcn_readfirstlane((int)threadIdx.x >> 6);
+    auto thread_id = [&]() __attribute__((always_inline)) {
+        int ln = (int)__builtin_amdgcn_mbcnt_hi(~0u, __builtin_amdgcn_mbcnt_lo(~0u, 0u)), w = wave_index;
+        asm volatile("" : "+v"(ln), "+s"(w));
+        return w * 64 + ln;
+    };
+    MK_STAMP(0);
+    const int n_layer = rows > 0 ? m.n_layer : 0;
+    auto window_phase = [&](const ModelLayerArgs &L, auto xregs_tag, const f16x8 *xf, f16x8 *cf) __attribute__((always_inline)) {
+        const int tid = thread_id();
+        Qkv2Args q;
+        q.x = m.x; q.w = L.wqkv; q.qs = nullptr; q.sc = nullptr; q.bias = L.bqkv; q.cu = m.cu; q.groups = RAGGED ? m.groups : nullptr; q.n_groups = nullptr;
+        q.out = m.ctx; q.n_head = m.n_head; q.n_sent = m.n_sent; q.spw = 1; q.slot_mask = m.slot_mask;
+        qkv_attention2_body<2 * NT, NT, GW_F16, !RAGGED, decltype(xregs_tag)::value, !RAGGED>(q, smem, window, tid, xf, cf);
+    };
+    auto tail_phase = [&](const ModelLayerArgs &L, f16x8 (&xf)[8 * NT], const f16x8 *cf) __attribute__((always_inline)) {
+        const int tid = thread_id();
+        TailArgs t;
+        t.ctx = m.ctx; t.x = m.x; t.wo = L.wo; t.w1p = L.w1p; t.w2p = L.w2p;
+        t.wo_qs = t.w1_qs = t.w2_qs = nullptr; t.wo_sc = t.w1_sc = t.w2_sc = nullptr;
+        t.bo = L.bo; t.g1 = L.g1; t.be1 = L.be1; t.b1 = L.b1; t.b2 = L.b2; t.g2 = L.g2; t.be2 = L.be2; t.out = m.x; t.I = m.I;
+        layer_tail_body<NT, GW_F16, RAGGED, !RAGGED, !RAGGED>(t, smem, tok0, rows, tid, xf, cf);
+    };
+    auto hand_over = [&]() __attribute__((always_inline)) {
+        __builtin_amdgcn_fence(__ATOMIC_RELEASE, "workgroup");
+        asm volatile("s_waitcnt vmcnt(0) lgkmcnt(0)\n\ts_barrier" ::: "memory");
+        __builtin_amdgcn_fence(__ATOMIC_ACQUIRE, "workgroup");
+    };
+    if constexpr (RAGGED) {
+        for (int l = 0; l < n_layer; ++l) {
+            f16x8 none[8 * NT];
+            window_phase(m.layer[l], std::false_type{}, nullptr, nullptr);
+            hand_over();
+            MK_STAMP(1 + 2 * l);
+            tail_phase(m.layer[l], none, nullptr);
+            hand_over();
+            MK_STAMP(2 + 2 * l);
+        }
+    } else {
+        f16x8 cf[8 * NT];
+        if constexpr (EMBED) {
+            f16x8 xf0[8 * NT];
+            if (wave_index >= 4) {
+                int ln = (int)__builtin_amdgcn_mbcnt_hi(~0u, __builtin_amdgcn_mbcnt_lo(~0u, 0u));
+                asm volatile("" : "+v"(ln));
+                const ModelEmbedArgs &e = static_cast<const ModelEmbedArgs &>(m);
+                embed_ln_fragments<8 * NT, EMBED - 1>(e.word, e.type, e.pos, e.ge, e.bee, e.tokens, e.n_vocab, window, wave_index & 3, ln, m.x, xf0);
+                asm volatile("s_waitcnt vmcnt(0)" ::: "memory");
+            } else {
+#pragma unroll
+                for (int q = 0; q < 8 * NT; ++q) asm volatile("" : "=v"(xf0[q]));
+            }
+            if (n_layer > 0) window_phase(m.layer[0], std::true_type{}, xf0, cf);
+            else hand_over();
+        } else
+        if (n_layer > 0) window_phase(m.layer[0], std::false_type{}, nullptr, cf);
+        for (int l = 0; l < n_layer; ++l) {
+            hand_over();
+            MK_STAMP(1 + 2 * l);
+            f16x8 xf[8 * NT];
+            tail_phase(m.layer[l], xf, cf);
+            hand_over();
+            MK_STAMP(2 + 2 * l);
+            if (l + 1 < n_layer) window_phase(m.layer[l + 1], std::true_type{}, xf, cf);
+            else {
+#pragma unroll
+                for (int q = 0; q < 8 * NT; ++q) asm volatile("" : "=v"(cf[q]));
+            }
+        }
+    }
+    if (m.pooled) {
+        const int tid = thread_id();
+        for (int j = 0; j < count; ++j) {
+            const int b = first + j, t0 = m.cu[b];
+            int n = m.cu[b + 1] - t0;
+            if (!RAGGED && (t0 != tok0 || n != 128)) n = -1;
+            if constexpr (POOL_MODES) pool_normalize_sentence(m.x, t0, n, b, 128 * NT, m.max_len, m.status, m.pooled, (float *)smem, tid, tid < 256, m.pool_mode);
+            else pool_normalize_sentence<false, false>(m.x, t0, n, b, 128 * NT, m.max_len, m.status, m.pooled, (float *)smem, tid, tid < 256);
+            __syncthreads();
+        }
+    }
+    MK_STAMP(1 + 2 * n_layer);
diff --git a/bert.cpp_amd/csrc/options.cpp b/bert.cpp_amd/csrc/options.cpp
--- a/bert.cpp_amd/csrc/options.cpp
+++ b/bert.cpp_amd/csrc/options.cpp
@@ -29,6 +29,7 @@
     else if (key == "qkv2") qkv2 = value != "0";
     else if (key == "gemm256") gemm256 = value != "0";
     else if (key == "ln_fold") ln_fold = value != "0";
+    else if (key == "embed_fold") embed_fold = value != "0";
     else if (key == "tail") tail = value != "0";
     else if (key == "latency") latency = value != "0";
     else if (key == "stage_kernel") stage_kernel = value != "0";
@@ -50,6 +51,7 @@
     static const char *const same_as_key[][2] = {
         {"BERT_HIP_LATENCY", "latency"}, {"BERT_HIP_LATENCY", "latency_tokens"},
         {"BERT_HIP_LN_FOLD", "ln_fold"},
+        {"BERT_HIP_EMBED_FOLD", "embed_fold"},
         {"BERT_HIP_CHUNK_TOKENS", "chunk_tokens"}, {"BERT_HIP_WINDOW_SLOTS", "window_slots"},
         {"BERT_HIP_F32", "f32"},
         {"BERT_HIP_POOLING", "pooling"}, {"BERT_HIP_NORMALIZE", "normalize"},
diff --git a/bert.cpp_amd/csrc/options.h b/bert.cpp_amd/csrc/options.h
--- a/bert.cpp_amd/csrc/options.h
+++ b/bert.cpp_amd/csrc/options.h
@@ -11,6 +11,7 @@
     bool gemm_naive = false, attn_naive = false;
     bool qkv2 = true, gemm256 = true, tail = true;
     bool ln_fold = true;
+    bool embed_fold = true;
     bool latency = true;
     bool q4_expand = true;
     bool f32_exact = true;
diff --git a/bert.cpp_amd/csrc/profiler.h b/bert.cpp_amd/csrc/profiler.h
--- a/bert.cpp_amd/csrc/profiler.h
+++ b/bert.cpp_amd/csrc/profiler.h
@@ -17,6 +17,7 @@
     ~LaunchProfiler();
 
     void enable(bool on) { profiling_ = on; }
+    bool enabled() const { return profiling_; }
     void set_replay(const std::string &value);
     void begin_pass() { replay_done_ = false; }
     void count_family(const std::string &family) { if (profiling_ && replay_name_.empty()) families_[family] += 1; }
diff --git a/bert.cpp_amd/pybert.py b/bert.cpp_amd/pybert.py
--- a/bert.cpp_amd/pybert.py
+++ b/bert.cpp_amd/pybert.py
@@ -35,7 +35,7 @@
     "bert_hip_test_pool",
     "bert_hip_test_model_digest", "bert_hip_test_pack_weight", "bert_hip_test_parse_devices", "bert_hip_test_gather_runs",
     "bert_hip_test_encode_groups", "bert_hip_test_tokenize_pack", "bert_hip_test_index_header",
-    "bert_hip_test_build_lists",
+    "bert_hip_test_build_lists", "bert_hip_test_poison_x", "bert_hip_test_embed_folded",
 ]
 TEST_LIB_PATH = LIB_PATH[:-3] + "_test.so"
 
@@ -183,6 +183,10 @@
     L.bert_hip_test_gather_runs.argtypes = [i32p, i32, C.c_int64, i32p]
     L.bert_hip_test_encode_groups.restype = i32
     L.bert_hip_test_encode_groups.argtypes = [i32, i32p, i32]
+    L.bert_hip_test_poison_x.restype = i32
+    L.bert_hip_test_poison_x.argtypes = [vp]
+    L.bert_hip_test_embed_folded.restype = i32
+    L.bert_hip_test_embed_folded.argtypes = [vp]
     L.bert_hip_test_tokenize_pack.restype = i32
     L.bert_hip_test_tokenize_pack.argtypes = [vp, i32, i32, C.POINTER(C.c_char_p), i32p, i32p, i32p, i32p, i32]
     L.bert_hip_test_index_header.restype = i32
```

Result: no change. 343,500 sentences/s (-0.4%).
